# pdegenhardt/MinCostFlow

Hardware: AMD Instinct MI355X
Metric: pivots/sec + solve ms, NETGEN 100k-node/300k-arc; arc-scan GB/s vs HBM peak (higher is better)
Workload: dtype int64

## Files before the change

### include/mcf_hip.h

```cpp
#ifndef MCF_HIP_H
#define MCF_HIP_H

#include <stdint.h>

#ifdef __cplusplus
extern "C" {
#endif

#define MCF_API __attribute__((visibility("default")))

typedef enum mcf_status {
    MCF_OK = 0,
    MCF_ERR_INVALID = -1,
    MCF_ERR_NO_DEVICE = -2,
    MCF_ERR_HIP = -3,
    MCF_ERR_OVERFLOW = -4,
    MCF_ERR_TIMEOUT = -5,
    MCF_ERR_STATE = -6,
    MCF_ERR_IO = -7,
    MCF_ERR_COMM = -8
} mcf_status;

typedef enum mcf_pivot_rule { MCF_RULE_FIRST_ELIGIBLE = 0, MCF_RULE_BEST_ELIGIBLE = 1, MCF_RULE_BLOCK_SEARCH = 2,
                              MCF_RULE_CANDIDATE_LIST = 3, MCF_RULE_ALTERING_LIST = 4 } mcf_pivot_rule;
// ... 85 lines not shown
                                  const int32_t *target, const int64_t *cost);

MCF_API int mcf_engine_check_reduced_costs(mcf_engine *e, int64_t *mismatches, int32_t *first_arc);
MCF_API int mcf_engine_can_renumber(mcf_engine *e, int32_t *yes);
MCF_API int mcf_engine_renumber_nodes(mcf_engine *e, const int32_t *new_of);

MCF_API int mcf_engine_find_entering(mcf_engine *e, int32_t *found, int32_t *arc, int64_t *reduced_cost);
MCF_API int mcf_engine_search_begin(mcf_engine *e);
MCF_API int mcf_engine_search_end(mcf_engine *e, int32_t *found, int32_t *arc, int64_t *reduced_cost);

#define MCF_COLLECT_FIRST_N 0
#define MCF_COLLECT_BLOCKS 1
typedef struct mcf_collect_request {
    int32_t next_arc;
    int32_t mode;
    int32_t limit;
    int32_t block_size;
    int32_t head_length;
    int32_t survivors;
} mcf_collect_request;
MCF_API int mcf_engine_collect_eligible(mcf_engine *e, const mcf_collect_request *rq, int32_t capacity, int32_t *count, int32_t *arcs,
                                        int64_t *reduced_costs, int32_t *end_arc, int64_t *arcs_scanned);

typedef struct mcf_candidate {
    int64_t reduced_cost;
    uint32_t pos;
    int32_t arc;
    int64_t range_cost;
    uint32_t range_pos;
    int32_t range_arc;
} mcf_candidate;
MCF_API int mcf_engine_find_entering_local(mcf_engine *e, mcf_candidate *out);
MCF_API int mcf_engine_search_end_local(mcf_engine *e, mcf_candidate *out);
MCF_API int mcf_engine_resolve(mcf_engine *e, int32_t count, const mcf_candidate *all, int32_t *found,
                               int32_t *arc, int64_t *reduced_cost);
MCF_API int mcf_resolve_candidates(int32_t rule, int32_t semantics, int32_t vector_width, int32_t search_arc_num, int32_t block_size, int32_t *next_arc,
                                   int32_t count, const mcf_candidate *all, int32_t *found, int32_t *arc, int64_t *reduced_cost);
MCF_API int mcf_shard_range(int32_t search_arc_num, int32_t rank, int32_t world, int32_t *begin, int32_t *end);

MCF_API int mcf_engine_park(mcf_engine *e);
MCF_API int mcf_engine_get_next_arc(mcf_engine *e, int32_t *next_arc);
MCF_API int mcf_engine_set_next_arc(mcf_engine *e, int32_t next_arc);
MCF_API int mcf_engine_get_block_size(mcf_engine *e, int32_t *block_size);
MCF_API int mcf_engine_set_block_config(mcf_engine *e, const mcf_block_config *c, int32_t graph_node_count);

MCF_API int mcf_engine_download_pi(mcf_engine *e, int64_t *pi_out );
MCF_API int mcf_engine_download_state(mcf_engine *e, int8_t *state_out );

typedef struct mcf_engine_stats {
    int64_t searches;
    int64_t scan_launches;
    int64_t update_launches;
    int64_t inline_updates;
    int64_t potential_nodes;
    int64_t arcs_scanned;
    int64_t timed_scans;
    double timed_scan_ns;
    double host_wait_ns;
    double host_launch_ns;
    int32_t scan_workgroups, scan_threads;
    int64_t bytes_per_scan;
    int64_t resident;
    int64_t resident_launches;
    int64_t resident_requests;
    double resident_scan_ns;
    double resident_kernel_ns;
    int64_t candidates;
    int64_t host_decided;
    int64_t arcs_checked;
    int32_t initial_block_size, current_block_size;
    int32_t comm_ranks;
    int32_t reserved;
    int64_t async_refreshes;
    int64_t scan_bytes_read;
    int64_t rc_layout;
    int64_t rc_recomputes;
    int64_t renumberings;
    int64_t heap_compactions;
    int64_t rc_reloads_in_grid;
    int64_t shift_grid;
    int64_t shift_lists;
    int64_t mirror_uploads;
    double phase_shift_ns, phase_values_ns, phase_scan_ns;
} mcf_engine_stats;
MCF_API int mcf_engine_get_stats(mcf_engine *e, mcf_engine_stats *out);
MCF_API int mcf_engine_reset_stats(mcf_engine *e);

MCF_API int mcf_engine_bench_scan(mcf_engine *e, int32_t reps, int32_t cold, int64_t flush_bytes,
                                  double *avg_ns, double *min_ns);

MCF_API int mcf_engine_bench_update(mcf_engine *e, int32_t count, int32_t reps, double *avg_ns, double *min_ns, int64_t *bytes);

MCF_API int mcf_engine_bench_search(mcf_engine *e, int32_t reps, double *avg_ns, double *min_ns);

MCF_API int mcf_comm_unique_id(uint8_t id_out[128]);
MCF_API int mcf_engine_comm_init(mcf_engine *e, const uint8_t id[128], int32_t rank, int32_t world);
MCF_API int mcf_engine_find_entering_sharded(mcf_engine *e, int32_t *found, int32_t *arc, int64_t *reduced_cost);

typedef struct mcf_exchange mcf_exchange;
MCF_API int mcf_exchange_open(mcf_exchange **out, const char *name, int32_t rank, int32_t world);
MCF_API void mcf_exchange_close(mcf_exchange *x);
MCF_API int mcf_exchange_all_gather(mcf_exchange *x, const mcf_candidate *mine, mcf_candidate *all );


typedef struct mcf_ns mcf_ns;

MCF_API int mcf_ns_create(mcf_ns **out, int32_t node_count, int32_t arc_count, const int32_t *source, const int32_t *target);
MCF_API void mcf_ns_destroy(mcf_ns *s);
MCF_API int mcf_ns_set_arc_bounds(mcf_ns *s, int32_t arc, int64_t lower, int64_t upper);
MCF_API int mcf_ns_set_arc_cost(mcf_ns *s, int32_t arc, int64_t cost);
MCF_API int mcf_ns_set_node_supply(mcf_ns *s, int32_t node, int64_t supply);
MCF_API int mcf_ns_set_problem(mcf_ns *s, const int64_t *lower, const int64_t *upper, const int64_t *cost, const int64_t *supply);
MCF_API int mcf_ns_set_supply_type(mcf_ns *s, int32_t type);
MCF_API int mcf_ns_set_pivot_rule(mcf_ns *s, int32_t rule);
MCF_API int mcf_ns_set_list_pivot_rule(mcf_ns *s, int32_t rule);
MCF_API int mcf_ns_enable_optimized_pivot(mcf_ns *s, int32_t enable);
MCF_API int mcf_ns_set_vector_width(mcf_ns *s, int32_t vector_width);
MCF_API int mcf_ns_set_optimization_config(mcf_ns *s, const mcf_block_config *config);
MCF_API int mcf_ns_enable_optimizations(mcf_ns *s, int32_t flags);
MCF_API int mcf_ns_set_auto_configuration(mcf_ns *s, int32_t enable);
MCF_API int mcf_ns_set_device(mcf_ns *s, int32_t device, int32_t int_width ,
                              int32_t block_size , int32_t engine_flags);
MCF_API int mcf_ns_set_device_share(mcf_ns *s, int32_t resident_workgroups);
MCF_API int mcf_ns_set_sharding(mcf_ns *s, const uint8_t nccl_id[128], int32_t rank, int32_t world);

MCF_API int mcf_ns_set_sharding_host(mcf_ns *s, const char *exchange_name, int32_t rank, int32_t world);
MCF_API int mcf_ns_set_shard_group(mcf_ns *s, int32_t shards, const int32_t *devices);

MCF_API int mcf_ns_prepare(mcf_ns *s);
MCF_API int mcf_ns_solve(mcf_ns *s, int32_t *status);
MCF_API int mcf_ns_status(mcf_ns *s, int32_t *status);
MCF_API int mcf_ns_get_flow(mcf_ns *s, int32_t arc, int64_t *flow);
MCF_API int mcf_ns_get_potential(mcf_ns *s, int32_t node, int64_t *potential);
MCF_API int mcf_ns_get_total_cost(mcf_ns *s, int64_t *cost);
MCF_API int mcf_ns_get_flows(mcf_ns *s, int64_t *flow_out );
MCF_API int mcf_ns_get_potentials(mcf_ns *s, int64_t *pi_out );
MCF_API int mcf_ns_get_arc_upper_bound(mcf_ns *s, int32_t arc, int64_t *upper);

typedef struct mcf_ns_metrics {
    int64_t iterations;
    double total_solve_us, pivot_search_us, tree_update_us, potential_update_us;
    double setup_us;
    double loop_us;
    int32_t search_arc_num, block_size, int_width, reserved;
    int64_t degenerate_pivots;
    int64_t potential_nodes;
    mcf_engine_stats engine;
    int32_t initial_block_size, final_block_size;
    int64_t total_arcs_checked;
    double average_arcs_checked_per_pivot;
    int32_t baseline_iterations;
    int32_t config_flags;
    double iteration_ratio;
    int32_t reference_selects_cached_pivot;
    int32_t reserved2;
} mcf_ns_metrics;
MCF_API int mcf_ns_get_metrics(mcf_ns *s, mcf_ns_metrics *out);
typedef struct mcf_list_rule_stats {
    int32_t rule;
    int32_t list_length;
    int32_t minor_limit;
    int32_t block_size;
    int32_t head_length;
    int32_t reserved;
    int64_t searches;
    int64_t major_scans;
    int64_t host_answered;
    int64_t device_arcs_read;
    int64_t lemon_arcs_scanned;
// ... 430 lines not shown
```

### mincostflow_amd/_lib.py

```python
from __future__ import annotations

import ctypes as C
import importlib.util
import os
import re
import sys
import warnings

import numpy as np

_HERE = os.path.dirname(os.path.abspath(__file__))
LIB_PATH = os.path.join(_HERE, "libmcf_hip.so")

RULE_FIRST_ELIGIBLE, RULE_BEST_ELIGIBLE, RULE_BLOCK_SEARCH, RULE_CANDIDATE_LIST, RULE_ALTERING_LIST = 0, 1, 2, 3, 4
COLLECT_FIRST_N, COLLECT_BLOCKS = 0, 1
SEM_PLAIN, SEM_OPTIMIZED = 1, 2
VECTOR_DEFAULT, VECTOR_NONE = 0, -1
SUPPLY_GEQ, SUPPLY_LEQ = 0, 1
NOT_SOLVED, OPTIMAL, INFEASIBLE, UNBOUNDED, UNBALANCED = 0, 1, 2, 3, 4
STATE_UPPER, STATE_TREE, STATE_LOWER = -1, 0, 1
INF_CAP = np.iinfo(np.int64).max
ENGINE_SAMPLE_KERNEL_TIME, ENGINE_TIME_EVERY_KERNEL, ENGINE_NO_INLINE_UPDATE, ENGINE_RESIDENT, ENGINE_DISPATCH, ENGINE_CANDIDATES = 1, 2, 4, 8, 16, 32
ENGINE_SHARE_DEVICE = 64
ENGINE_NO_CANDIDATES = 128
ERR_INVALID, ERR_NO_DEVICE, ERR_HIP, ERR_OVERFLOW, ERR_TIMEOUT, ERR_STATE, ERR_IO, ERR_COMM = -1, -2, -3, -4, -5, -6, -7, -8


class McfError(RuntimeError):
    def __init__(self, code: int, message: str):
        super().__init__(f"mcf_hip error {code}: {message}")
        self.code = code


class EngineDesc(C.Structure):
    _fields_ = [(n, C.c_int32) for n in ("node_count", "arc_capacity", "search_arc_num", "int_width", "rule", "semantics",
                                         "block_size", "device", "shard_begin", "shard_end", "scan_workgroups", "flags", "resident_workgroups", "vector_width")]


class Candidate(C.Structure):
    _fields_ = [("reduced_cost", C.c_int64), ("pos", C.c_uint32), ("arc", C.c_int32),
                ("range_cost", C.c_int64), ("range_pos", C.c_uint32), ("range_arc", C.c_int32)]

    def __init__(self, reduced_cost=0, pos=0xFFFFFFFF, arc=-1, range_cost=0, range_pos=0xFFFFFFFF, range_arc=-1):
        super().__init__(reduced_cost, pos, arc, range_cost, range_pos, range_arc)


class EngineStats(C.Structure):
    _fields_ = [("searches", C.c_int64), ("scan_launches", C.c_int64), ("update_launches", C.c_int64),
                ("inline_updates", C.c_int64), ("potential_nodes", C.c_int64), ("arcs_scanned", C.c_int64),
                ("timed_scans", C.c_int64), ("timed_scan_ns", C.c_double), ("host_wait_ns", C.c_double),
                ("host_launch_ns", C.c_double), ("scan_workgroups", C.c_int32), ("scan_threads", C.c_int32),
                ("bytes_per_scan", C.c_int64), ("resident", C.c_int64), ("resident_launches", C.c_int64),
                ("resident_requests", C.c_int64), ("resident_scan_ns", C.c_double), ("resident_kernel_ns", C.c_double), ("candidates", C.c_int64),
                ("host_decided", C.c_int64), ("arcs_checked", C.c_int64), ("initial_block_size", C.c_int32), ("current_block_size", C.c_int32),
                ("comm_ranks", C.c_int32), ("reserved", C.c_int32), ("async_refreshes", C.c_int64), ("scan_bytes_read", C.c_int64), ("rc_layout", C.c_int64), ("rc_recomputes", C.c_int64), ("renumberings", C.c_int64), ("heap_compactions", C.c_int64), ("rc_reloads_in_grid", C.c_int64), ("shift_grid", C.c_int64), ("shift_lists", C.c_int64), ("mirror_uploads", C.c_int64),
                ("phase_shift_ns", C.c_double), ("phase_values_ns", C.c_double), ("phase_scan_ns", C.c_double)]

    def as_dict(self):
        return {n: getattr(self, n) for n, _ in self._fields_ if n != "reserved"}


OPT_NONE, OPT_ADAPTIVE_BLOCK_SIZE, OPT_SMALL_BLOCKS_FOR_DENSE, OPT_REDUCED_COST_CACHING = 0, 1, 2, 4


class BlockConfig(C.Structure):
    _fields_ = [("flags", C.c_int32), ("min_block_size", C.c_int32), ("max_block_size", C.c_int32), ("consecutive_hits_before_adapt", C.c_int32),
                ("min_block_size_ratio", C.c_double), ("block_size_growth_factor", C.c_double), ("block_size_shrink_factor", C.c_double),
                ("low_hit_rate_threshold", C.c_double), ("high_hit_rate_threshold", C.c_double)]

    def as_dict(self):
        return {n: getattr(self, n) for n, _ in self._fields_}


class NsMetrics(C.Structure):
    _fields_ = [("iterations", C.c_int64), ("total_solve_us", C.c_double), ("pivot_search_us", C.c_double),
                ("tree_update_us", C.c_double), ("potential_update_us", C.c_double), ("setup_us", C.c_double),
                ("loop_us", C.c_double), ("search_arc_num", C.c_int32),
                ("block_size", C.c_int32), ("int_width", C.c_int32), ("reserved", C.c_int32),
                ("degenerate_pivots", C.c_int64), ("potential_nodes", C.c_int64), ("engine", EngineStats),
                ("initial_block_size", C.c_int32), ("final_block_size", C.c_int32), ("total_arcs_checked", C.c_int64),
                ("average_arcs_checked_per_pivot", C.c_double), ("baseline_iterations", C.c_int32), ("config_flags", C.c_int32),
                ("iteration_ratio", C.c_double), ("reference_selects_cached_pivot", C.c_int32), ("reserved2", C.c_int32)]

    def as_dict(self):
        d = {n: getattr(self, n) for n, _ in self._fields_ if n not in ("engine", "reserved", "reserved2")}
        d["engine"] = self.engine.as_dict()
        return d


VALIDATION_KINDS = ("conservation", "lower", "upper", "slack_pos", "slack_neg", "node_dual", "node_slack", "objective", "dual_cost", "status")


class CollectRequest(C.Structure):
    _fields_ = [(n, C.c_int32) for n in ("next_arc", "mode", "limit", "block_size", "head_length", "survivors")]


class ListRuleStats(C.Structure):
    _fields_ = [("rule", C.c_int32), ("list_length", C.c_int32), ("minor_limit", C.c_int32), ("block_size", C.c_int32), ("head_length", C.c_int32),
                ("reserved", C.c_int32), ("searches", C.c_int64), ("major_scans", C.c_int64), ("host_answered", C.c_int64),
                ("device_arcs_read", C.c_int64), ("lemon_arcs_scanned", C.c_int64), ("collected", C.c_int64), ("collect_us", C.c_double)]

    def as_dict(self):
        return {n: getattr(self, n) for n, _ in self._fields_ if n != "reserved"}


class Validation(C.Structure):
    _fields_ = [("valid", C.c_int32), ("supply_type", C.c_int32), ("objective", C.c_int64), ("dual_cost", C.c_int64),
                ("errors", C.c_int64 * len(VALIDATION_KINDS)), ("first", C.c_int64 * len(VALIDATION_KINDS)),
                ("kernel_us", C.c_double), ("algorithmic_bytes", C.c_int64)]

    def as_dict(self):
        return {"valid": int(self.valid), "supply_type": int(self.supply_type), "objective": int(self.objective), "dual_cost": int(self.dual_cost),
                "errors": dict(zip(VALIDATION_KINDS, map(int, self.errors))), "first": dict(zip(VALIDATION_KINDS, map(int, self.first))),
                "kernel_us": float(self.kernel_us), "algorithmic_bytes": int(self.algorithmic_bytes)}


class BatchDesc(C.Structure):
    _fields_ = [("device", C.c_int32), ("pivot_rule", C.c_int32), ("semantics", C.c_int32), ("reserved", C.c_int32), ("pivot_limit", C.c_int64),
                ("pivots_per_launch", C.c_int32), ("trace_capacity", C.c_int32), ("flags", C.c_int32)]


class BatchStats(C.Structure):
    _fields_ = [("instances", C.c_int64), ("lds_instances", C.c_int64), ("global_instances", C.c_int64), ("launches", C.c_int64),
                ("total_pivots", C.c_int64), ("workspace_bytes", C.c_int64), ("lds_bytes_max", C.c_int64), ("kernel_ns", C.c_double), ("host_ns", C.c_double)]

    def as_dict(self):
        return {n: getattr(self, n) for n, _ in self._fields_}


class BatchResolveStats(C.Structure):
    _fields_ = [("warm_instances", C.c_int64), ("cold_instances", C.c_int64), ("untouched_instances", C.c_int64), ("launches", C.c_int64),
                ("total_pivots", C.c_int64), ("bytes_uploaded", C.c_int64), ("bytes_downloaded", C.c_int64), ("kernel_ns", C.c_double), ("host_ns", C.c_double)]

    def as_dict(self):
        return {n: getattr(self, n) for n, _ in self._fields_}


BATCH_MAX_ARCS, BATCH_MAX_NODES, BATCH_MAX_INSTANCES, BATCH_SHARDED = 65536, 32768, 65536, 1
MEM_HOST, MEM_DEVICE = 0, 1
# ... 119 lines not shown


class RBatchDiagnoseIo(C.Structure):
    _fields_ = UBatchDiagnoseIo._fields_


class UBatchDiagnoseStats(C.Structure):
    _fields_ = [(name, C.c_int64) for name in ("instances", "none", "feasible", "cut", "open", "bounds", "lds_instances", "global_instances", "levels",
                                               "frontier_nodes", "inc_entries")] + \
               [("kernel_ns", C.c_double), ("bytes_up", C.c_int64), ("bytes_down", C.c_int64)]

    def as_dict(self):
        return {n: getattr(self, n) for n, _ in self._fields_}


class ProblemStruct(C.Structure):
    _fields_ = [("node_count", C.c_int32), ("arc_count", C.c_int32), ("source", C.POINTER(C.c_int32)),
                ("target", C.POINTER(C.c_int32)), ("lower", C.POINTER(C.c_int64)), ("upper", C.POINTER(C.c_int64)),
                ("cost", C.POINTER(C.c_int64)), ("supply", C.POINTER(C.c_int64))]


_i32p = np.ctypeslib.ndpointer(np.int32, flags="C_CONTIGUOUS")
_i64p = np.ctypeslib.ndpointer(np.int64, flags="C_CONTIGUOUS")


class _i64p_or_null(_i64p):
    @classmethod
    def from_param(cls, obj):
        return None if obj is None else _i64p.from_param(obj)


_i8p = np.ctypeslib.ndpointer(np.int8, flags="C_CONTIGUOUS")
_u8p = np.ctypeslib.ndpointer(np.uint8, flags="C_CONTIGUOUS")
_P = C.POINTER

SIGNATURES = {
    "mcf_last_error": (C.c_char_p, []),
    "mcf_version": (C.c_char_p, []),
    "mcf_device_count": (C.c_int, []),
    "mcf_device_compute_units": (C.c_int, [C.c_int32]),
    "mcf_engine_create": (C.c_int, [_P(C.c_void_p), _P(EngineDesc)]),
    "mcf_engine_destroy": (None, [C.c_void_p]),
    "mcf_engine_upload": (C.c_int, [C.c_void_p, _i32p, _i32p, _i64p, _i8p, _i64p]),
    "mcf_engine_patch_state": (C.c_int, [C.c_void_p, C.c_int32, _i32p, _i8p]),
    "mcf_engine_update_potential": (C.c_int, [C.c_void_p, C.c_int32, _i32p, C.c_int64]),
    "mcf_engine_set_potential": (C.c_int, [C.c_void_p, C.c_int32, _i32p, _i64p]),
    "mcf_engine_append_potential": (C.c_int, [C.c_void_p, C.c_int32, _i32p, _i64p]),
    "mcf_engine_bind_potentials": (C.c_int, [C.c_void_p, C.c_void_p]),
    "mcf_engine_shift_potential": (C.c_int, [C.c_void_p, C.c_int32, _i32p, _i64p_or_null, C.c_int64]),
    "mcf_engine_shift_potential_runs": (C.c_int, [C.c_void_p, C.c_int32, _i32p, _i32p, C.c_int64]),
    "mcf_engine_reload_threshold": (C.c_int, [C.c_void_p, C.POINTER(C.c_int32)]),
    "mcf_engine_reload_potentials": (C.c_int, [C.c_void_p, C.c_int32]),
    "mcf_engine_patch_arcs": (C.c_int, [C.c_void_p, C.c_int32, _i32p, _i32p, _i32p, _i64p]),
    "mcf_engine_can_renumber": (C.c_int, [C.c_void_p, _P(C.c_int32)]),
    "mcf_engine_check_reduced_costs": (C.c_int, [C.c_void_p, _P(C.c_int64), _P(C.c_int32)]),
    "mcf_ns_check_reduced_costs": (C.c_int, [C.c_void_p, _P(C.c_int64)]),
    "mcf_engine_renumber_nodes": (C.c_int, [C.c_void_p, _i32p]),
    "mcf_engine_find_entering": (C.c_int, [C.c_void_p, _P(C.c_int32), _P(C.c_int32), _P(C.c_int64)]),
    "mcf_engine_search_begin": (C.c_int, [C.c_void_p]),
    "mcf_engine_search_end": (C.c_int, [C.c_void_p, _P(C.c_int32), _P(C.c_int32), _P(C.c_int64)]),
    "mcf_engine_find_entering_local": (C.c_int, [C.c_void_p, _P(Candidate)]),
    "mcf_engine_collect_eligible": (C.c_int, [C.c_void_p, _P(CollectRequest), C.c_int32, _P(C.c_int32), C.c_void_p, C.c_void_p,
                                              _P(C.c_int32), _P(C.c_int64)]),
    "mcf_engine_search_end_local": (C.c_int, [C.c_void_p, _P(Candidate)]),
    "mcf_exchange_open": (C.c_int, [_P(C.c_void_p), C.c_char_p, C.c_int32, C.c_int32]),
    "mcf_exchange_close": (None, [C.c_void_p]),
    "mcf_exchange_all_gather": (C.c_int, [C.c_void_p, _P(Candidate), _P(Candidate)]),
    "mcf_engine_resolve": (C.c_int, [C.c_void_p, C.c_int32, _P(Candidate), _P(C.c_int32), _P(C.c_int32), _P(C.c_int64)]),
    "mcf_resolve_candidates": (C.c_int, [C.c_int32, C.c_int32, C.c_int32, C.c_int32, C.c_int32, _P(C.c_int32), C.c_int32, _P(Candidate),
                                        _P(C.c_int32), _P(C.c_int32), _P(C.c_int64)]),
    "mcf_shard_range": (C.c_int, [C.c_int32, C.c_int32, C.c_int32, _P(C.c_int32), _P(C.c_int32)]),
    "mcf_engine_park": (C.c_int, [C.c_void_p]),
    "mcf_engine_get_next_arc": (C.c_int, [C.c_void_p, _P(C.c_int32)]),
    "mcf_engine_set_next_arc": (C.c_int, [C.c_void_p, C.c_int32]),
    "mcf_engine_get_block_size": (C.c_int, [C.c_void_p, _P(C.c_int32)]),
    "mcf_block_config_default": (None, [_P(BlockConfig)]),
    "mcf_block_config_auto": (C.c_int, [_P(BlockConfig), C.c_int32, C.c_int32, _i32p, _i32p]),
    "mcf_block_initial_size": (C.c_int, [_P(BlockConfig), C.c_int32, C.c_int32, _P(C.c_int32), _P(C.c_int32)]),
    "mcf_block_adapt": (C.c_int, [_P(BlockConfig), C.c_int32, C.c_int64, _P(C.c_int32), _P(C.c_int32)]),
    "mcf_engine_set_block_config": (C.c_int, [C.c_void_p, _P(BlockConfig), C.c_int32]),
    "mcf_engine_download_pi": (C.c_int, [C.c_void_p, _i64p]),
    "mcf_engine_download_state": (C.c_int, [C.c_void_p, _i8p]),
    "mcf_engine_get_stats": (C.c_int, [C.c_void_p, _P(EngineStats)]),
    "mcf_engine_reset_stats": (C.c_int, [C.c_void_p]),
    "mcf_engine_bench_scan": (C.c_int, [C.c_void_p, C.c_int32, C.c_int32, C.c_int64, _P(C.c_double), _P(C.c_double)]),
    "mcf_engine_bench_search": (C.c_int, [C.c_void_p, C.c_int32, _P(C.c_double), _P(C.c_double)]),
    "mcf_engine_bench_update": (C.c_int, [C.c_void_p, C.c_int32, C.c_int32, _P(C.c_double), _P(C.c_double), _P(C.c_int64)]),
    "mcf_comm_unique_id": (C.c_int, [_u8p]),
    "mcf_engine_comm_init": (C.c_int, [C.c_void_p, _u8p, C.c_int32, C.c_int32]),
    "mcf_engine_find_entering_sharded": (C.c_int, [C.c_void_p, _P(C.c_int32), _P(C.c_int32), _P(C.c_int64)]),
    "mcf_ns_create": (C.c_int, [_P(C.c_void_p), C.c_int32, C.c_int32, _i32p, _i32p]),
    "mcf_ns_destroy": (None, [C.c_void_p]),
    "mcf_ns_set_arc_bounds": (C.c_int, [C.c_void_p, C.c_int32, C.c_int64, C.c_int64]),
    "mcf_ns_set_arc_cost": (C.c_int, [C.c_void_p, C.c_int32, C.c_int64]),
    "mcf_ns_set_node_supply": (C.c_int, [C.c_void_p, C.c_int32, C.c_int64]),
    "mcf_ns_set_problem": (C.c_int, [C.c_void_p, C.c_void_p, C.c_void_p, C.c_void_p, C.c_void_p]),
    "mcf_ns_set_supply_type": (C.c_int, [C.c_void_p, C.c_int32]),
    "mcf_ns_set_pivot_rule": (C.c_int, [C.c_void_p, C.c_int32]),
    "mcf_ns_set_list_pivot_rule": (C.c_int, [C.c_void_p, C.c_int32]),
    "mcf_ns_enable_optimized_pivot": (C.c_int, [C.c_void_p, C.c_int32]),
    "mcf_ns_set_vector_width": (C.c_int, [C.c_void_p, C.c_int32]),
    "mcf_ns_set_optimization_config": (C.c_int, [C.c_void_p, _P(BlockConfig)]),
    "mcf_ns_enable_optimizations": (C.c_int, [C.c_void_p, C.c_int32]),
    "mcf_ns_set_auto_configuration": (C.c_int, [C.c_void_p, C.c_int32]),
    "mcf_ns_set_device": (C.c_int, [C.c_void_p, C.c_int32, C.c_int32, C.c_int32, C.c_int32]),
    "mcf_ns_set_device_share": (C.c_int, [C.c_void_p, C.c_int32]),
    "mcf_ns_set_sharding": (C.c_int, [C.c_void_p, _u8p, C.c_int32, C.c_int32]),
    "mcf_ns_set_sharding_host": (C.c_int, [C.c_void_p, C.c_char_p, C.c_int32, C.c_int32]),
    "mcf_ns_set_shard_group": (C.c_int, [C.c_void_p, C.c_int32, _i32p]),
    "mcf_ns_prepare": (C.c_int, [C.c_void_p]),
    "mcf_ns_solve": (C.c_int, [C.c_void_p, _P(C.c_int32)]),
    "mcf_ns_status": (C.c_int, [C.c_void_p, _P(C.c_int32)]),
    "mcf_ns_get_flow": (C.c_int, [C.c_void_p, C.c_int32, _P(C.c_int64)]),
    "mcf_ns_get_potential": (C.c_int, [C.c_void_p, C.c_int32, _P(C.c_int64)]),
    "mcf_ns_get_total_cost": (C.c_int, [C.c_void_p, _P(C.c_int64)]),
    "mcf_ns_get_flows": (C.c_int, [C.c_void_p, _i64p]),
    "mcf_ns_get_potentials": (C.c_int, [C.c_void_p, _i64p]),
    "mcf_ns_get_arc_upper_bound": (C.c_int, [C.c_void_p, C.c_int32, _P(C.c_int64)]),
    "mcf_ns_get_metrics": (C.c_int, [C.c_void_p, _P(NsMetrics)]),
    "mcf_ns_get_list_rule_stats": (C.c_int, [C.c_void_p, _P(ListRuleStats)]),
    "mcf_ns_set_pivot_limit": (C.c_int, [C.c_void_p, C.c_int64]),
    "mcf_ns_set_trace": (C.c_int, [C.c_void_p, C.c_void_p, C.c_int64]),
    "mcf_ns_get_trace_length": (C.c_int, [C.c_void_p, _P(C.c_int64)]),
    "mcf_ns_begin": (C.c_int, [C.c_void_p, _P(C.c_int32)]),
    "mcf_ns_apply_pivot": (C.c_int, [C.c_void_p, C.c_int32, _P(C.c_int32)]),
    "mcf_ns_finish": (C.c_int, [C.c_void_p, _P(C.c_int32)]),
    "mcf_ns_replay": (C.c_int, [C.c_void_p, _i32p, C.c_int64, C.c_int32, C.c_double]),
    "mcf_ns_check_thread_breaks": (C.c_int, [C.c_void_p, _P(C.c_int64)]),
    "mcf_ns_internal": (C.c_int, [C.c_void_p, _P(C.c_int32), _P(C.c_int32), _P(_P(C.c_int32)), _P(_P(C.c_int32)),
                                  _P(_P(C.c_int64)), _P(_P(C.c_int8)), _P(_P(C.c_int64))]),
    "mcf_ns_tree": (C.c_int, [C.c_void_p, _P(_P(C.c_int32)), _P(_P(C.c_int32)), _P(_P(C.c_int32)), _P(_P(C.c_int8)), _P(_P(C.c_int64)), _P(_P(C.c_int64))]),
    "mcf_ns_last_pivot": (C.c_int, [C.c_void_p, _P(C.c_int32), _P(C.c_int32), _P(C.c_int8), _P(C.c_int32),
                                    _P(_P(C.c_int32)), _P(C.c_int64)]),
    "mcf_validator_create": (C.c_int, [_P(C.c_void_p), C.c_int32, C.c_int32, C.c_int32]),
    "mcf_validator_destroy": (None, [C.c_void_p]),
    "mcf_validator_upload": (C.c_int, [C.c_void_p] + [C.c_void_p] * 8),
    "mcf_validator_run": (C.c_int, [C.c_void_p, C.c_int32, C.c_int64, _P(Validation)]),
    "mcf_ns_validate": (C.c_int, [C.c_void_p, _P(Validation)]),
    "mcf_batch_create": (C.c_int, [_P(C.c_void_p), _P(BatchDesc)]),
    "mcf_batch_destroy": (None, [C.c_void_p]),
    "mcf_batch_add": (C.c_int, [C.c_void_p, C.c_int32, C.c_int32, C.c_void_p, C.c_void_p, C.c_void_p, C.c_void_p, C.c_void_p, C.c_void_p, C.c_int32, _P(C.c_int32)]),
    "mcf_batch_solve": (C.c_int, [C.c_void_p]),
    "mcf_batch_run_on_host": (C.c_int, [C.c_void_p]),
    "mcf_batch_get_status": (C.c_int, [C.c_void_p, C.c_int32, _P(C.c_int32)]),
    "mcf_batch_get_total_cost": (C.c_int, [C.c_void_p, C.c_int32, _P(C.c_int64)]),
    "mcf_batch_get_flows": (C.c_int, [C.c_void_p, C.c_int32, C.c_void_p]),
    "mcf_batch_get_potentials": (C.c_int, [C.c_void_p, C.c_int32, C.c_void_p]),
    "mcf_batch_get_pivots": (C.c_int, [C.c_void_p, C.c_int32, _P(C.c_int64)]),
    "mcf_batch_get_trace": (C.c_int, [C.c_void_p, C.c_int32, C.c_void_p, C.c_int64, _P(C.c_int64)]),
    "mcf_batch_get_stats": (C.c_int, [C.c_void_p, _P(BatchStats)]),
    "mcf_batch_set_costs": (C.c_int, [C.c_void_p, C.c_int32, C.c_void_p]),
    "mcf_batch_resolve": (C.c_int, [C.c_void_p]),
    "mcf_batch_rerun_on_host": (C.c_int, [C.c_void_p]),
    "mcf_batch_get_resolve_stats": (C.c_int, [C.c_void_p, _P(BatchResolveStats)]),
    "mcf_ubatch_create": (C.c_int, [_P(C.c_void_p), _P(UBatchDesc)]),
    "mcf_ubatch_destroy": (None, [C.c_void_p]),
    "mcf_ubatch_solve": (C.c_int, [C.c_void_p, _P(UBatchIo)]),
    "mcf_ubatch_resolve": (C.c_int, [C.c_void_p, _P(UBatchIo)]),
    "mcf_ubatch_run_on_host": (C.c_int, [C.c_void_p, _P(UBatchIo)]),
    "mcf_ubatch_rerun_on_host": (C.c_int, [C.c_void_p, _P(UBatchIo)]),
    "mcf_ubatch_get_stats": (C.c_int, [C.c_void_p, _P(UBatchStats)]),
    "mcf_ubatch_resolve_data": (C.c_int, [C.c_void_p, _P(UBatchIo)]),
    "mcf_ubatch_rerun_data_on_host": (C.c_int, [C.c_void_p, _P(UBatchIo)]),
    "mcf_ubatch_get_redata_stats": (C.c_int, [C.c_void_p, _P(UBatchRedataStats)]),
    "mcf_ubatch_validate": (C.c_int, [C.c_void_p, _P(UBatchCheckIo), _P(UBatchCheckSummary)]),
    "mcf_ubatch_validate_on_host": (C.c_int, [C.c_void_p, _P(UBatchCheckIo), _P(UBatchCheckSummary)]),
# ... 105 lines not shown
```

### mincostflow_amd/csrc/candidate_cache.hip.h

```cpp
#pragma once

static_assert(kCandNone == kNone, "the state's 'no arc' is the kernels'");
constexpr int kCandRefreshLow = 12;
constexpr int kCandMaxAvgDegree = 24;

inline const int64_t *cand_pi(const mcf_engine *e) { return e->ext_pi ? e->ext_pi : e->pi.data(); }
inline CandGraph cand_graph(const mcf_engine *e)
{
    return CandGraph{e->adj_start.data(), e->adj.data(), e->h_src.data(), e->h_tgt.data(), e->h_cost.data(), e->h_state.data(), cand_pi(e)};
}

inline void cand_note_node(mcf_engine *e, int u, bool sigma_known = false, int64_t sigma = 0)
{
    if (e->rc_mode) {
        if (sigma_known) e->rc_sync.push_back(mcf_engine::NodeShift{u, sigma});
        else e->rc_shift_unknown = true;
    }
    if (e->blind_count > 0 && e->blind_epoch == e->cand_now) e->blind_sets = 2;
    if (cand_state_note_node(e, u, e->adj_start.data())) e->sync_nodes.push_back(u);
}
inline void cand_note_arc(mcf_engine *e, int a)
{
    if (cand_state_note_arc(e, a)) e->sync_arcs.push_back(a);
}
// ... 26 lines not shown
        for (int r = 0; r < n_runs; ++r) for (int k = 0; k < length[r]; ++k) e->pend_node.push_back(first[r] + k);
        e->pend_val.resize(e->pend_node.size(), 0);
        e->blind_count = e->pend_node.size();
    } else {
        e->blind_lazy = true;
        for (int r = 0; r < n_runs; ++r)
            for (int32_t at = 0; at < length[r]; at += kShiftRunMax) {
                e->blind_runs.push_back((uint32_t)(first[r] + at));
                e->blind_runs.push_back((uint32_t)std::min<int32_t>(kShiftRunMax, length[r] - at));
            }
        e->blind_count += (size_t)total;
    }
    if (e->async_posted && cand_records_ready(e, 0)) { const int rc = cand_collect(e, e->async_at); if (rc) return rc; }
    shift_stream(e);
    return MCF_OK;
}

inline int cand_note_nodes_blind(mcf_engine *e, int32_t count, const int32_t *nodes, const int64_t *values, bool continuation)
{
    if (e->blind_lazy) {
        if (e->shift_streamed > 0) { const int rc = resident_stop(e); if (rc) return rc; }
        cand_materialise_blind(e);
    }
    e->pivot_overflow = true;
    if (e->blind_count == 0) { e->blind_epoch = e->cand_now; e->blind_sets = 0; }
    if (!continuation) {
        e->blind_sets += 1;
        if (e->blind_sets > 1 && e->stream_lines > 0) { const int rc = resident_stop(e); if (rc) return rc; }
    }
    e->pend_node.insert(e->pend_node.end(), nodes, nodes + count);
    if (values) e->pend_val.insert(e->pend_val.end(), values, values + count);
    else {
        const size_t at = e->pend_val.size();
        e->pend_val.resize(at + (size_t)count);
        if (!e->shift_grid) for (int i = 0; i < count; ++i) e->pend_val[at + i] = e->ext_pi[nodes[i]];
    }
    e->blind_count = e->pend_node.size();
    if (e->async_posted && cand_records_ready(e, 0)) { const int rc = cand_collect(e, e->async_at); if (rc) return rc; }
    if (e->shift_grid) shift_stream(e);
    else resident_stream(e);
    return MCF_OK;
}

bool cand_decide(mcf_engine *e, Key *k)
{
    mcf_engine::CandKey win;
    if (!cand_decide(static_cast<CandState *>(e), &win)) return false;
    k->c = win.p == kNone ? 0 : win.c;
    k->r = 0;
    k->p = win.p;
    return true;
}

int cand_build_patches(mcf_engine *e)
{
    const int64_t *pi = cand_pi(e);
    const size_t n_b = e->blind_count, n_s = e->sync_nodes.size();
    const bool blind_current = n_b == 0 || (e->blind_epoch == e->cand_now && e->blind_sets <= 1);
    const bool squeeze = (int64_t)n_b + (int64_t)n_s > e->patch_capacity;
    if ((!blind_current || squeeze) && e->stream_lines > 0) { const int rc = resident_stop(e); if (rc) return rc; }
    if (squeeze) {
        e->pend_node.insert(e->pend_node.end(), e->sync_nodes.begin(), e->sync_nodes.end());
        std::sort(e->pend_node.begin(), e->pend_node.end());
        e->pend_node.erase(std::unique(e->pend_node.begin(), e->pend_node.end()), e->pend_node.end());
        e->pend_val.resize(e->pend_node.size());
        for (size_t i = 0; i < e->pend_node.size(); ++i) e->pend_val[i] = pi[e->pend_node[i]];
    } else {
        if (!blind_current) for (size_t i = 0; i < n_b; ++i) e->pend_val[i] = pi[e->pend_node[i]];
        e->pend_node.resize(n_b + n_s);
        e->pend_val.resize(n_b + n_s);
        for (size_t i = 0; i < n_s; ++i) { e->pend_node[n_b + i] = e->sync_nodes[i]; e->pend_val[n_b + i] = pi[e->sync_nodes[i]]; }
    }
    e->pend_arc.assign(e->sync_arcs.begin(), e->sync_arcs.end());
    e->pend_state.resize(e->pend_arc.size());
    for (size_t i = 0; i < e->pend_arc.size(); ++i) e->pend_state[i] = e->h_state[e->pend_arc[i]];
    e->sync_nodes.clear();
    e->sync_arcs.clear();
    blind_clear(e);
    e->rc_sync.clear();
    e->rc_shift_unknown = false;
    return MCF_OK;
}

bool cand_records_ready(const mcf_engine *e, int g)
{
    const volatile Slot *rec = e->h_slots + (size_t)g * kCandRecords;
    for (int r = 0; r < kCandRecords; ++r) { const int64_t c = rec[r].c; const uint32_t q = rec[r].p; if (rec[r].tag != record_tag(e->seq, c, q)) return false; }
    return true;
}

int cand_collect(mcf_engine *e, uint32_t at)
{
    const double t0 = (double)__rdtsc();
    double t0_wall = 0;
    const volatile Slot *slots = e->h_slots;
    e->cand_records.clear();
    mcf_engine::CandKey thr{0, kNone};
    for (int g = 0; g < e->res_grid; ++g) {
        const volatile Slot *rec = slots + (size_t)g * kCandRecords;
        uint64_t spins = 0;
        while (!cand_records_ready(e, g)) {
            _mm_pause();
            if (e->resident_running && (spins & 0xFFF) == 0xFFF && ((const volatile uint32_t *)e->h_exit)[0] != 0) {
                if (((const volatile uint32_t *)e->h_exit)[0] == kExitPartial) {
                    (void)resident_join(e, false);
                    e->resident_running = false;
                    resident_slot_release(e);
                    return mcf::fail(MCF_ERR_TIMEOUT, "the resident grid could not meet at its grid-wide barrier while a list was being applied (are its workgroups all resident?): the device arrays are undefined");
                }
                int rc = resident_restart(e);
                if (rc) return rc;
            }
            if ((++spins & 0xFFFFF) == 0) {
                const hipError_t q = hipStreamQuery(e->res_stream ? e->res_stream : e->stream);
                if (q != hipSuccess && q != hipErrorNotReady) return mcf::fail(MCF_ERR_HIP, "resident grid failed: %s", hipGetErrorString(q));
                if (t0_wall == 0) t0_wall = mcf::now_ns();
                else if (mcf::now_ns() - t0_wall > 20e9) return mcf::fail(MCF_ERR_TIMEOUT, "no answer from the device after 20 s (workgroup %d of %d)", g, e->res_grid);
            }
        }
        std::atomic_thread_fence(std::memory_order_acquire);
        for (int r = 0; r < kCandPerGroup; ++r)
            if (rec[r].p != kNone) e->cand_records.push_back(mcf_engine::CandKey{rec[r].c, rec[r].p});
        if (rec[kCandPerGroup].p != kNone) {
            const mcf_engine::CandKey t{rec[kCandPerGroup].c, rec[kCandPerGroup].p};
            if (thr.p == kNone || cand_key_less(t, thr)) thr = t;
        }
    }
    e->wait_ticks += (double)__rdtsc() - t0;
    cand_install(e, cand_graph(e), e->cand_records.data(), e->cand_records.size(), thr, at);
    e->tk_collect += (double)__rdtsc() - t0;
    return MCF_OK;
}

int cand_post_rc(mcf_engine *e)
{
    const bool reload = e->reload_pi && e->d_ext_pi != nullptr && (int64_t)e->sync_arcs.size() <= e->mailbox_max_st;
    if (reload) {
        pend_clear_potentials(e);
        e->sync_nodes.clear(); e->rc_sync.clear(); e->rc_shift_unknown = false;
        blind_clear(e);
        e->reload_pi = false;
    }
    const size_t n_b = e->blind_count, n_s = e->rc_sync.size();
    const bool blind_ok = n_b == 0 || (e->pend_shift && e->blind_epoch == e->cand_now);
    const int64_t n_st = (int64_t)e->sync_arcs.size();
    const bool fast = !e->reload_pi && !e->rc_shift_unknown && blind_ok && (int64_t)(n_b + n_s) <= (int64_t)e->rc_list_max && n_st <= e->mailbox_max_st;
    if (fast) {
        e->pend_node.resize(n_b + n_s);
        e->pend_val.resize(n_b + n_s);
        for (size_t i = 0; i < n_b; ++i) e->pend_val[i] = e->pend_sigma;
        for (size_t i = 0; i < n_s; ++i) { e->pend_node[n_b + i] = e->rc_sync[i].node; e->pend_val[n_b + i] = e->rc_sync[i].shift; }
        e->pend_arc.assign(e->sync_arcs.begin(), e->sync_arcs.end());
        e->pend_state.resize(e->pend_arc.size());
        for (size_t i = 0; i < e->pend_arc.size(); ++i) e->pend_state[i] = e->h_state[e->pend_arc[i]];
        e->sync_nodes.clear(); e->sync_arcs.clear(); e->rc_sync.clear();
        blind_clear(e);
    } else {
        if (int rcb = cand_build_patches(e)) return rcb;
        int rc = resident_stop(e);
        if (!rc) rc = flush_pending(e);
        if (rc) return rc;
    }
    next_request_keep_prev(e);
    int rc = resident_start(e, e->prev_seq);
    if (rc) return rc;
    resident_post(e, e->seq, reload ? kCmdReload : kCmdScan, fast);
    if (reload) e->st.rc_reloads_in_grid += 1;
    if (fast && (!e->pend_node.empty() || !e->pend_arc.empty())) e->st.inline_updates += 1;
    pend_clear(e);
    e->posted_at = e->cand_now;
    e->st.arcs_scanned += e->end - e->begin;
    return MCF_OK;
}


int device_sync_from_mirrors(mcf_engine *e)
{
    const int64_t *pi = cand_pi(e);
    HIP_TRY(hipMemcpyAsync(e->d_pi, pi, sizeof(int64_t) * (size_t)e->d.node_count, hipMemcpyHostToDevice, e->stream));
    HIP_TRY(hipMemcpyAsync(e->d_state, e->h_state.data() + e->begin, (size_t)(e->end - e->begin), hipMemcpyHostToDevice, e->stream));
    HIP_TRY(hipStreamSynchronize(e->stream));
    pend_clear(e);
    e->pend_shift = false;
    e->sync_nodes.clear(); e->sync_arcs.clear(); e->rc_sync.clear(); e->rc_shift_unknown = false;
    blind_clear(e); e->blind_sets = 0;
    e->shift_streamed = 0;
    e->reload_pi = false;
    e->st.mirror_uploads += 1;
    return MCF_OK;
}

void shift_write_lines(mcf_engine *e, int from, int to, size_t n, bool runs, uint32_t seq)
{
    const int per_line = runs ? kShiftPairsPerLine : kShiftNodesPerLine;
    MailboxLine line;
    for (int l = from; l < to; ++l) {
        memset(line.w, 0, sizeof(line.w));
        for (int k = 0; k < per_line && (size_t)l * per_line + k < n; ++k) {
            const size_t i = (size_t)l * per_line + k;
            if (runs) { line.w[2 * k] = e->blind_runs[2 * i]; line.w[2 * k + 1] = e->blind_runs[2 * i + 1]; }
            else line.w[k] = (uint32_t)e->pend_node[i];
        }
        line.w[15] = seq;
        mailbox_write_line(e->mailbox + e->shift_base + 16 * (size_t)l, line.w);
    }
}

void shift_post_request(mcf_engine *e, uint32_t seq, uint32_t cmd, size_t val_lo, size_t n_shift, int64_t sigma, bool with_patches, bool runs = false)
{
    const int n_val = with_patches ? (int)(e->pend_node.size() - val_lo) : 0, n_st = with_patches ? (int)e->pend_arc.size() : 0;
    const ValueEntries vals{e->pend_node.data(), e->pend_val.data(), val_lo + 1, n_val > 1 ? n_val - 1 : 0};
    const StateEntries sts{e->pend_arc.data(), e->pend_state.data(), 2, n_st > 2 ? n_st - 2 : 0};
    const MailboxLine line1 = mailbox_encode_entries(e->mailbox, vals, sts, seq);
    if (with_patches) {
        const int per_line = runs ? kShiftPairsPerLine : kShiftNodesPerLine;
        shift_write_lines(e, e->shift_streamed, (int)((n_shift + per_line - 1) / per_line), n_shift, runs, seq);
        e->shift_streamed = 0;
    }
    MailboxLine h = request_header(e, seq, cmd, n_st, n_val, val_lo);
    h.w[kShHdrValues] = (uint32_t)n_val;
    h.w[kShHdrShift] = with_patches ? (uint32_t)n_shift : 0u;
    h.w[kShHdrRuns] = with_patches && runs ? 1u : 0u;
    h.w[kShHdrSigma] = (uint32_t)(uint64_t)sigma;
    h.w[kShHdrSigma + 1] = (uint32_t)((uint64_t)sigma >> 32);
    mailbox_publish(e->mailbox, kPollReplicas, h, vals.n + sts.n > 0 ? &line1 : nullptr);
}
void shift_post(mcf_engine *e, uint32_t seq, uint32_t cmd, bool) { shift_post_request(e, seq, cmd, 0, 0, 0, false); }

constexpr int kShiftStreamMinLines = 96;
void shift_stream(mcf_engine *e)
{
    if (e->async_posted || e->blind_epoch != e->cand_now || e->blind_sets > 1 || !e->pend_shift) return;
    if (!e->resident_running || e->in_flight != mcf_engine::kNoSearch) return;
    const bool runs = e->blind_lazy;
    const int complete = runs ? (int)(e->blind_runs.size() / 2 / kShiftPairsPerLine) : (int)(e->blind_count / kShiftNodesPerLine);
    if (complete - e->shift_streamed < kShiftStreamMinLines || complete > e->max_shift_lines) return;
    const uint32_t next_seq = peek_request(e);
    shift_write_lines(e, e->shift_streamed, complete, runs ? e->blind_runs.size() / 2 : e->blind_count, runs, next_seq);
    e->stream_sub += 1;
    if (e->stream_sub == 0) e->stream_sub = 1;
    MailboxLine h = request_header(e, next_seq, runs ? kCmdApplyRuns : kCmdApply);
    h.w[kShHdrShift] = (uint32_t)complete;
    h.w[kShHdrApplySub] = e->stream_sub;
    mailbox_publish(e->mailbox, kPollReplicas, h, nullptr);
    e->shift_streamed = complete;
    e->stream_lines = complete;
}

int cand_post_shift(mcf_engine *e)
{
    if (!e->resident_running) {
        const int rc = resident_start(e, e->seq);
        if (rc) return rc;
    }
    if (e->reload_pi) {
        if (!e->d_ext_pi || e->shift_streamed > 0 || (int64_t)e->sync_arcs.size() > (int64_t)e->mailbox_max_st) {
            int rc = resident_stop(e);
            if (!rc) rc = resident_start(e, e->seq);
            if (rc) return rc;
        }
    }
    if (e->reload_pi) {
        pend_clear_potentials(e);
        e->sync_nodes.clear();
        blind_clear(e);
        e->pend_arc.assign(e->sync_arcs.begin(), e->sync_arcs.end());
        e->pend_state.resize(e->pend_arc.size());
        for (size_t i = 0; i < e->pend_arc.size(); ++i) e->pend_state[i] = e->h_state[e->pend_arc[i]];
        next_request_keep_prev(e);
        shift_post_request(e, e->seq, kCmdReload, 0, 0, 0, true);
        e->st.rc_reloads_in_grid += 1;
        e->pend_arc.clear(); e->pend_state.clear();
        e->sync_arcs.clear();
        e->stream_lines = 0;
        e->reload_pi = false;
        e->posted_at = e->cand_now;
        e->st.arcs_scanned += e->end - e->begin;
        return MCF_OK;
    }
    for (int attempt = 0; attempt < 2; ++attempt) {
        const size_t n_b = e->blind_count, n_s = e->sync_nodes.size();
        const bool blind_current = n_b == 0 || (e->blind_epoch == e->cand_now && e->blind_sets <= 1);
        const size_t n_pairs = e->blind_lazy ? e->blind_runs.size() / 2 : 0;
        const bool as_shift = n_b > 0 && blind_current && e->pend_shift &&
                              (e->blind_lazy ? n_pairs <= (size_t)e->max_shift_lines * kShiftPairsPerLine : n_b <= (size_t)e->max_shift_lines * kShiftNodesPerLine);
        const bool fits = (int64_t)(as_shift ? n_s : n_b + n_s) <= (int64_t)e->patch_capacity && (int64_t)e->sync_arcs.size() <= (int64_t)e->mailbox_max_st;
        if ((!as_shift && e->shift_streamed > 0) || !fits) {
            int rc = resident_stop(e);
            if (!rc) rc = resident_start(e, e->seq);
            if (rc) return rc;
            continue;
        }
        const int64_t *pi = cand_pi(e);
        const bool runs = as_shift && e->blind_lazy;
        if (!as_shift) cand_materialise_blind(e);
        const size_t base = runs ? 0 : n_b, val_lo = as_shift ? base : 0;
        if (!as_shift) for (size_t i = 0; i < n_b; ++i) e->pend_val[i] = pi[e->pend_node[i]];
        e->pend_node.resize(base + n_s);
        e->pend_val.resize(base + n_s);
        for (size_t i = 0; i < n_s; ++i) { e->pend_node[base + i] = e->sync_nodes[i]; e->pend_val[base + i] = pi[e->sync_nodes[i]]; }
        e->pend_arc.assign(e->sync_arcs.begin(), e->sync_arcs.end());
        e->pend_state.resize(e->pend_arc.size());
        for (size_t i = 0; i < e->pend_arc.size(); ++i) e->pend_state[i] = e->h_state[e->pend_arc[i]];
        next_request_keep_prev(e);
        shift_post_request(e, e->seq, kCmdScan, val_lo, as_shift ? (runs ? n_pairs : n_b) : 0, e->pend_sigma, true, runs);
        if (!e->pend_node.empty() || !e->pend_arc.empty()) e->st.inline_updates += 1;
        if (as_shift) e->st.shift_lists += 1;
        pend_clear(e);
        e->sync_nodes.clear(); e->sync_arcs.clear();
        blind_clear(e);
        e->stream_lines = 0;
        e->posted_at = e->cand_now;
        e->st.arcs_scanned += e->end - e->begin;
        return MCF_OK;
    }
    return mcf::fail(MCF_ERR_STATE, "cand_post_shift: the request does not fit an empty mailbox");
}

int cand_post(mcf_engine *e)
{
    if (e->shift_grid) return cand_post_shift(e);
    if (e->rc_mode) return cand_post_rc(e);
    if (int rcb = cand_build_patches(e)) return rcb;
    if ((int)e->pend_arc.size() > e->mailbox_max_st) {
        int rc = resident_stop(e);
        if (!rc) rc = flush_pending(e);
        if (rc) return rc;
    }
    next_request_keep_prev(e);
    int rc = resident_start(e, e->prev_seq);
    if (rc) return rc;
    resident_post(e, e->seq, kCmdScan, true);
    if (!e->pend_node.empty() || !e->pend_arc.empty()) e->st.inline_updates += 1;
    pend_clear(e);
    e->posted_at = e->cand_now;
    e->st.arcs_scanned += e->end - e->begin;
    return MCF_OK;
}

void cand_build_adjacency(mcf_engine *e)
{
    const int n = e->d.node_count, m_s = e->d.search_arc_num;
    const int32_t *source = e->h_src.data(), *target = e->h_tgt.data();
    const int lo = e->begin, hi = std::min(e->end, m_s);
    e->adj_start.assign(n + 1, 0);
    for (int a = lo; a < hi; ++a) { e->adj_start[source[a] + 1]++; if (target[a] != source[a]) e->adj_start[target[a] + 1]++; }
    for (int u = 0; u < n; ++u) e->adj_start[u + 1] += e->adj_start[u];
    e->adj.assign(e->adj_start[n], mcf_engine::AdjEnt{0, 0u, 0});
    e->adj_pos.assign((size_t)2 * m_s, -1);
    std::vector<int32_t> fill(e->adj_start.begin(), e->adj_start.end() - 1);
    for (int a = lo; a < hi; ++a) {
        const uint32_t st_bits = (uint32_t)(e->h_state[a] + 1) << 29;
        e->adj_pos[2 * (size_t)a] = fill[source[a]];
        e->adj[fill[source[a]]++] = mcf_engine::AdjEnt{a, (uint32_t)target[a] | st_bits, e->h_cost[a]};
        if (target[a] != source[a]) {
            e->adj_pos[2 * (size_t)a + 1] = fill[target[a]];
            e->adj[fill[target[a]]++] = mcf_engine::AdjEnt{a, (uint32_t)source[a] | st_bits | 0x80000000u, e->h_cost[a]};
        }
    }
}
```

### mincostflow_amd/csrc/candidate_state.h

```cpp
#pragma once

#include <algorithm>
#include <cstdint>
#include <vector>

#include "common.h"

constexpr uint32_t kCandNone = 0xFFFFFFFFu;
constexpr int kCandMaxNodes = 256;
constexpr int64_t kCandDegreePerNode = 8;

struct CandState {
    struct AdjEnt { int32_t arc; uint32_t other; int64_t cost; };
    struct CandKey { int64_t c; uint32_t p; };
    struct HeapEnt { int64_t c; uint32_t p; uint32_t at; int32_t u, v; };

    bool cand_valid = false;
    mcf::hvec<uint32_t> node_at, arc_at;
    uint32_t cand_now = 1;
    uint32_t snap_at = 0;
    uint32_t heap_gap = 0;
    std::vector<HeapEnt> heap;
    std::vector<int32_t> pivot_nodes, pivot_arcs;
    int64_t pivot_degree = 0;
    bool pivot_overflow = false;
    std::vector<CandKey> cand_list;
    std::vector<int32_t> cand_ends;
    size_t cand_ptr = 0;
    bool tp_ok = false, hd_ok = false;
    int32_t tp_a = -1, tp_u = -1, tp_v = -1, hd_a = -1, hd_u = -1, hd_v = -1;
    uint32_t tp_at = 0;
    size_t hd_ptr = 0;
    CandKey cand_thr{0, kCandNone};
    bool async_posted = false;
    size_t heap_compact_above = 1u << 18;
    int64_t n_heap_push = 0, n_heap_admit = 0, n_heap_pop = 0, n_heap_sweeps = 0;
};

struct CandGraph {
    const int32_t *adj_start;
    const CandState::AdjEnt *adj;
    const int32_t *src, *tgt;
    const int64_t *cost;
    const int8_t *state;
    const int64_t *pi;
};

inline bool cand_key_less(const CandState::CandKey &a, const CandState::CandKey &b) { return a.c < b.c || (a.c == b.c && a.p < b.p); }
struct CandHeapAfter {
    bool operator()(const CandState::HeapEnt &a, const CandState::HeapEnt &b) const { return b.c < a.c || (b.c == a.c && b.p < a.p); }
};

inline bool cand_state_note_node(CandState *e, int u, const int32_t *adj_start)
{
    if ((u == e->tp_u) | (u == e->tp_v)) e->tp_ok = false;
    if ((u == e->hd_u) | (u == e->hd_v)) e->hd_ok = false;
    if (e->node_at[u] == e->cand_now) return false;
    e->node_at[u] = e->cand_now;
    if (!e->pivot_overflow) {
        e->pivot_nodes.push_back(u);
        e->pivot_degree += adj_start[u + 1] - adj_start[u];
        if ((int)e->pivot_nodes.size() > kCandMaxNodes || e->pivot_degree > kCandDegreePerNode * kCandMaxNodes) e->pivot_overflow = true;
    }
    return true;
}
inline bool cand_state_note_arc(CandState *e, int a)
{
    if (a == e->tp_a) e->tp_ok = false;
    if (a == e->hd_a) e->hd_ok = false;
    if (e->arc_at[a] == e->cand_now) return false;
    e->arc_at[a] = e->cand_now;
    e->pivot_arcs.push_back(a);
    return true;
}

inline bool cand_heap_current(const CandState *e, const CandState::HeapEnt &t)
{
    return ((int)(e->arc_at[t.p] <= t.at) & (int)(e->node_at[t.u] <= t.at) & (int)(e->node_at[t.v] <= t.at)) != 0;
}

inline bool cand_admit_all(const CandState *e) { return e->async_posted || !e->cand_valid || e->cand_thr.p == kCandNone; }

inline void cand_sweep_heap(CandState *e, bool install)
{
    if (e->heap.empty()) return;
    size_t keep = 0;
    if (install) {
        const bool all = e->cand_thr.p == kCandNone;
        for (size_t i = 0; i < e->heap.size(); ++i) {
            const CandState::HeapEnt &t = e->heap[i];
            if (t.at > e->snap_at && (all || cand_key_less(CandState::CandKey{t.c, t.p}, e->cand_thr))) e->heap[keep++] = t;
        }
    } else {
        for (size_t i = 0; i < e->heap.size(); ++i)
            if (cand_heap_current(e, e->heap[i])) e->heap[keep++] = e->heap[i];
    }
    e->heap.resize(keep);
    std::make_heap(e->heap.begin(), e->heap.end(), CandHeapAfter());
    e->n_heap_sweeps += 1;
}

inline void cand_push(CandState *e, const CandGraph &g, int a)
{
    const int st = g.state[a];
    if (st == 0) return;
    const int64_t *pi = g.pi;
    const int32_t u = g.src[a], v = g.tgt[a];
    const int64_t d = g.cost[a] + pi[u] - pi[v];
    const int64_t rc = st > 0 ? d : -d;
    if (rc >= 0) return;
    e->n_heap_push += 1;
    if (!cand_admit_all(e) && !cand_key_less(CandState::CandKey{rc, (uint32_t)a}, e->cand_thr)) return;
    e->n_heap_admit += 1;
    e->heap.push_back(CandState::HeapEnt{rc, (uint32_t)a, e->cand_now, u, v});
    std::push_heap(e->heap.begin(), e->heap.end(), CandHeapAfter());
}

inline void cand_absorb_pivot(CandState *e, const CandGraph &g)
{
    if (e->pivot_overflow) {
// ... 2 lines not shown
        const int64_t *pi = g.pi;
        const uint32_t now = e->cand_now;
        const bool admit_all = cand_admit_all(e);
        const CandState::CandKey thr = e->cand_thr;
        int64_t offered = 0, admitted = 0;
        for (int u : e->pivot_nodes)
            for (int i = g.adj_start[u], hi = g.adj_start[u + 1]; i < hi; ++i) {
                const CandState::AdjEnt &x = g.adj[i];
                __builtin_prefetch(&pi[x.other & 0x1FFFFFFFu]);
            }
        for (int u : e->pivot_nodes) {
            const int64_t pu = pi[u];
            for (int i = g.adj_start[u], hi = g.adj_start[u + 1]; i < hi; ++i) {
                const CandState::AdjEnt &x = g.adj[i];
                const int st = (int)((x.other >> 29) & 3u) - 1;
                if (st == 0) continue;
                const int32_t other = (int32_t)(x.other & 0x1FFFFFFFu);
                const int64_t po = pi[other];
                const int64_t d = (x.other >> 31) ? x.cost + po - pu : x.cost + pu - po;
                const int64_t rc = st > 0 ? d : -d;
                if (rc >= 0) continue;
                offered += 1;
                if (!admit_all && !cand_key_less(CandState::CandKey{rc, (uint32_t)x.arc}, thr)) continue;
                admitted += 1;
                e->heap.push_back(CandState::HeapEnt{rc, (uint32_t)x.arc, now, u, other});
                std::push_heap(e->heap.begin(), e->heap.end(), CandHeapAfter());
            }
        }
        e->n_heap_push += offered;
        e->n_heap_admit += admitted;
        for (int a : e->pivot_arcs) cand_push(e, g, a);
    }
    e->pivot_nodes.clear();
    e->pivot_arcs.clear();
    e->pivot_degree = 0;
    e->pivot_overflow = false;
    if (e->heap.size() > e->heap_compact_above) cand_sweep_heap(e, false);
}

inline bool cand_decide(CandState *e, CandState::CandKey *out)
{
    if (!e->cand_valid || e->snap_at < e->heap_gap) return false;
    CandState::CandKey best_d{0, kCandNone};
    while (!e->heap.empty()) {
        const CandState::HeapEnt &t = e->heap.front();
        const uint32_t a = t.p;
        if (e->tp_ok && (int32_t)a == e->tp_a && t.at == e->tp_at) { best_d = CandState::CandKey{t.c, a}; break; }
        const bool after = t.at > e->snap_at;
        if (after && cand_heap_current(e, t)) {
            e->tp_ok = true; e->tp_a = (int32_t)a; e->tp_at = t.at; e->tp_u = t.u; e->tp_v = t.v;
            best_d = CandState::CandKey{t.c, a};
            break;
        }
        std::pop_heap(e->heap.begin(), e->heap.end(), CandHeapAfter());
        e->heap.pop_back();
        e->n_heap_pop += 1;
    }
    while (e->cand_ptr < e->cand_list.size()) {
        if (e->hd_ok && e->hd_ptr == e->cand_ptr) break;
        const uint32_t a = e->cand_list[e->cand_ptr].p;
        if (e->cand_ptr + 1 < e->cand_list.size()) {
            __builtin_prefetch(&e->arc_at[e->cand_list[e->cand_ptr + 1].p]);
            __builtin_prefetch(&e->node_at[e->cand_ends[2 * e->cand_ptr + 2]]);
            __builtin_prefetch(&e->node_at[e->cand_ends[2 * e->cand_ptr + 3]]);
        }
        const uint32_t t_arc = e->arc_at[a], t_src = e->node_at[e->cand_ends[2 * e->cand_ptr]], t_tgt = e->node_at[e->cand_ends[2 * e->cand_ptr + 1]];
        if ((t_arc <= e->snap_at) & (t_src <= e->snap_at) & (t_tgt <= e->snap_at)) {
            e->hd_ok = true; e->hd_ptr = e->cand_ptr; e->hd_a = (int32_t)a; e->hd_u = e->cand_ends[2 * e->cand_ptr]; e->hd_v = e->cand_ends[2 * e->cand_ptr + 1];
            break;
        }
        e->cand_ptr++;
    }
    CandState::CandKey win{0, kCandNone};
    if (e->cand_ptr < e->cand_list.size()) {
        win = e->cand_list[e->cand_ptr];
        if (best_d.p != kCandNone && cand_key_less(best_d, win)) win = best_d;
    } else if (e->cand_thr.p == kCandNone) {
        win = best_d;
    } else if (best_d.p != kCandNone && cand_key_less(best_d, e->cand_thr)) {
        win = best_d;
    } else {
        return false;
    }
    *out = win;
    return true;
}

inline void cand_install(CandState *e, const CandGraph &g, const CandState::CandKey *rec, size_t n, CandState::CandKey thr, uint32_t at)
{
    e->cand_thr = thr;
    e->cand_list.clear();
    for (size_t i = 0; i < n; ++i)
        if (thr.p == kCandNone || cand_key_less(rec[i], thr)) e->cand_list.push_back(rec[i]);
    std::sort(e->cand_list.begin(), e->cand_list.end(), cand_key_less);
    e->cand_ends.resize(2 * e->cand_list.size());
    for (size_t i = 0; i < e->cand_list.size(); ++i) { e->cand_ends[2 * i] = g.src[e->cand_list[i].p]; e->cand_ends[2 * i + 1] = g.tgt[e->cand_list[i].p]; }
    e->cand_ptr = 0;
    e->cand_valid = true;
    e->hd_ok = e->tp_ok = false;
    e->snap_at = at;
    e->async_posted = false;
    cand_sweep_heap(e, true);
}

inline void cand_reset(CandState *e)
{
    e->cand_valid = false;
    e->cand_list.clear();
    e->cand_ptr = 0;
    e->hd_ok = e->tp_ok = false;
    e->heap.clear();
    e->pivot_nodes.clear(); e->pivot_arcs.clear(); e->pivot_degree = 0; e->pivot_overflow = false;
    e->heap_gap = e->cand_now;
}

constexpr uint32_t kCandEpochWrap = 0xFFFFFF00u;
inline void cand_restart_epochs(CandState *e)
{
    std::fill(e->node_at.begin(), e->node_at.end(), 0u);
    std::fill(e->arc_at.begin(), e->arc_at.end(), 0u);
    const bool overflow = e->pivot_overflow;
    const std::vector<int32_t> pn = e->pivot_nodes, pa = e->pivot_arcs;
    cand_reset(e);
    e->cand_now = 1;
    e->snap_at = 0;
    e->heap_gap = 1;
    e->pivot_overflow = overflow;
    for (int u : pn) e->node_at[u] = 1;
    for (int a : pa) e->arc_at[a] = 1;
}

inline void cand_renumber(CandState *e, const int32_t *new_of, int n)
{
    mcf::hvec<uint32_t> at((size_t)n);
    for (int u = 0; u < n; ++u) at[new_of[u]] = e->node_at[u];
    std::copy(at.begin(), at.end(), e->node_at.begin());
    for (size_t i = 0; i < e->cand_ends.size(); ++i) e->cand_ends[i] = new_of[e->cand_ends[i]];
    for (auto &h : e->heap) { h.u = new_of[h.u]; h.v = new_of[h.v]; }
    e->tp_ok = e->hd_ok = false;
    for (int32_t &u : e->pivot_nodes) u = new_of[u];
}
```

### mincostflow_amd/csrc/engine.hip

```cpp
#include <hip/hip_runtime.h>
#include <hip/hip_ext.h>
#include <hsa/hsa.h>
#include <hsa/hsa_ext_amd.h>

#include <dlfcn.h>
#include <immintrin.h>

#include <algorithm>
#include <atomic>
#include <cmath>
#include <cstdio>
#include <cstring>
#include <map>
#include <mutex>
#include <vector>

#include "common.h"
#include "candidate_state.h"

#include "kernels.hip.h"
#include "collect.hip.h"

namespace {

// ... 76 lines not shown
    int rc_recompute_above = INT32_MAX;
    int rc_list_max = 0;
    bool pend_shift = false;
    int64_t pend_sigma = 0;
    bool no_pireg = false;
    int lds_grid = 0;
    uint32_t seq = 0;
    bool uploaded = false;
    mcf::hvec<int64_t> pi;
    bool mirror_valid = false;
    bool ext_pi_pinned = false;
    const int64_t *d_ext_pi = nullptr;
    uint32_t *d_barrier = nullptr;
    int32_t *d_node_map = nullptr;
    bool reload_pi = false;
    const int64_t *ext_pi = nullptr;
    int64_t max_abs_cost = 0;
    mcf::hvec<int32_t> pend_node, pend_arc, pend_state;
    mcf::hvec<int64_t> pend_val;
    struct Staging {
        int32_t *nodes = nullptr, *arcs = nullptr, *states = nullptr;
        int64_t *values = nullptr;
        void *d_nodes = nullptr, *d_arcs = nullptr, *d_states = nullptr, *d_values = nullptr;
        hipEvent_t done = nullptr;
        bool busy = false;
        int cap_nodes = 0;
    } stage[2];
    int stage_next = 0;
    static constexpr int kEvRing = 64;
    hipEvent_t ev_start[kEvRing]{}, ev_stop[kEvRing]{};
    int ev_head = 0, ev_tail = 0;
    mcf_engine_stats st{};
    void *comm = nullptr;
    int rank = 0, world = 1;
    mcf_candidate *d_cand_local = nullptr, *d_cand_all = nullptr, *h_cand_all = nullptr;
    struct XRec { uint64_t head; mcf_candidate c; uint64_t pad[2]; uint64_t tail; };
    XRec *x_send = nullptr, *x_recv = nullptr;
    void *d_x_send = nullptr, *d_x_recv = nullptr;
    hipStream_t comm_stream = nullptr;
    uint64_t x_seq = 0;
    bool comm_resident = false;
    bool resident_ok = false, resident_running = false, resident_reg = false;
    bool has_slot = false;
    int shift_reload_min = 0;
    bool shift_grid = false;
    uint32_t shift_base = 0;
    int max_shift_lines = 0;
    int cand_tiles = 1;
    int shift_streamed = 0;
    double wait_ticks = 0, launch_ticks = 0, cal_ns = 0, cal_ticks = 0;
    enum { kNoSearch = 0, kAnswered, kResidentSearch, kCandSearch, kDispatchSearch } in_flight = kNoSearch;
    Key answered{0, kNone, kNone};
    Key range_key{0, kNone, kNone};
    int vec = 0;
    bool in_flight_timed = false;
    int stream_lines = 0;
    uint32_t stream_sub = 0;
    uint32_t *mailbox = nullptr;
    int mailbox_lines = 0, mailbox_max_st = 0;
    uint32_t idle_ticks = 0;
    uint32_t prev_seq = 0;
    bool cand_on = false;
    mcf::hvec<int32_t> h_src, h_tgt;
    mcf::hvec<int64_t> h_cost;
    mcf::hvec<int8_t> h_state;
    mcf::hvec<int32_t> adj_start;
    mcf::hvec<AdjEnt> adj;
    mcf::hvec<int32_t> adj_pos;
    std::vector<int32_t> sync_nodes, sync_arcs;
    size_t blind_count = 0;
    std::vector<uint32_t> blind_runs;
    bool blind_lazy = false;
    uint32_t blind_epoch = 0;
    int blind_sets = 0;
    bool force_device_search = false;
    bool cand_appending = false;
    struct NodeShift { int32_t node; int64_t shift; };
    std::vector<NodeShift> rc_sync;
    bool rc_shift_unknown = false;
    bool call_shift_known = false;
    int64_t call_shift = 0;
    std::vector<CandState::CandKey> cand_records;
    uint32_t async_at = 0, posted_at = 0;
    int patch_capacity = 0;
    uint32_t cand_epoch0 = 1;
    bool cand_debug = false;
    double tk_absorb = 0, tk_decide = 0, tk_post = 0, tk_collect = 0, tk_probe = 0;
    int64_t n_sync_posts = 0, n_async_waits = 0, n_gap_pivots = 0, n_list_skip = 0;
    uint32_t *h_exit = nullptr, *d_exit = nullptr;
    int res_grid = 0, res_threads = kResidentThreads;
    hipEvent_t res_start = nullptr, res_stop = nullptr;
    void *d_flush = nullptr;
    size_t flush_bytes = 0;
    bool list_rule = false;
    std::vector<int32_t> pend_index;
    CollectTile *d_tiles = nullptr;
    CollectHeader *h_collect_hdr = nullptr, *d_collect_hdr = nullptr;
    CollectEntry *h_collect = nullptr, *d_collect = nullptr;
    int collect_cap = 0;
};

namespace {
inline void blind_clear(mcf_engine *e)
{
    e->blind_count = 0;
    e->blind_runs.clear();
    e->blind_lazy = false;
}

#include "engine_helpers.hip.h"

bool fits32(int64_t v) { return v >= INT32_MIN && v <= INT32_MAX; }

int drain_events(mcf_engine *e, bool all)
{
    while (e->ev_tail != e->ev_head) {
        const int i = e->ev_tail % mcf_engine::kEvRing;
        if (!all && hipEventQuery(e->ev_stop[i]) != hipSuccess) break;
        HIP_TRY(hipEventSynchronize(e->ev_stop[i]));
        float ms = 0.f;
        HIP_TRY(hipEventElapsedTime(&ms, e->ev_start[i], e->ev_stop[i]));
        e->st.timed_scans += 1;
        e->st.timed_scan_ns += (double)ms * 1e6;
        e->ev_tail++;
    }
    return MCF_OK;
}

template <typename T>
void fill_params(mcf_engine *e, ScanParams<T> &p, bool with_patches)
{
    p.src = e->d_src;
    p.tgt = e->d_tgt;
    p.cost = (const T *)e->d_cost;
    p.state = e->d_state;
    p.pi = (T *)e->d_pi;
    p.slots = e->slots_target ? e->slots_target : e->d_slots;
    p.orig = e->bucket_nodes > 0 ? e->d_orig : nullptr;
    p.base = e->begin;
    p.count_padded = e->count_padded;
    p.m_s = e->d.search_arc_num;
    const SearchHeader h = search_header(e);
    p.next_arc = h.next_arc;
    p.block_size = h.block_size;
    p.rstar = h.rstar;
    p.seq = e->seq;
    p.n_pi = 0;
    p.n_st = 0;
    if (with_patches) {
        p.n_pi = (int)e->pend_node.size();
        p.n_st = (int)e->pend_arc.size();
        for (int i = 0; i < p.n_pi; ++i) { p.pi_node[i] = e->pend_node[i]; p.pi_val[i] = (T)e->pend_val[i]; }
        for (int i = 0; i < p.n_st; ++i) { p.st_arc[i] = e->pend_arc[i]; p.st_val[i] = e->pend_state[i]; }
    }
}

void fill_rc_params(mcf_engine *e, RcParams &p, bool with_states)
{
    p.state_ro = e->d_state; p.state = e->d_state; p.rc = e->d_rc; p.slots = e->slots_target ? e->slots_target : e->d_slots;
    p.base = e->begin; p.count_padded = e->count_padded; p.m_s = e->d.search_arc_num;
    const SearchHeader h = search_header(e);
    p.next_arc = h.next_arc;
    p.block_size = h.block_size;
    p.rstar = h.rstar;
    p.seq = e->seq;
    p.n_st = 0;
// ... 408 lines not shown
    if (desc->int_width != 32 && desc->int_width != 64) return mcf::fail(MCF_ERR_INVALID, "int_width must be 32 or 64");
    if (desc->rule < 0 || desc->rule > 4) return mcf::fail(MCF_ERR_INVALID, "pivot rule %d does not exist (Types/PivotRule.cs:7-41)", desc->rule);
    const bool list_rule = desc->rule == MCF_RULE_CANDIDATE_LIST || desc->rule == MCF_RULE_ALTERING_LIST;
    if (list_rule && !((desc->shard_begin == 0 && desc->shard_end == 0) || (desc->shard_begin == 0 && desc->shard_end == desc->search_arc_num)))
        return mcf::fail(MCF_ERR_INVALID, "the list rules (3, 4) scan the whole search range: no arc shards");
    if (desc->semantics != MCF_SEM_PLAIN && desc->semantics != MCF_SEM_OPTIMIZED) return mcf::fail(MCF_ERR_INVALID, "bad semantics %d", desc->semantics);
    if (desc->vector_width != MCF_VECTOR_DEFAULT && desc->vector_width != MCF_VECTOR_NONE && desc->vector_width != 2 && desc->vector_width != 4 && desc->vector_width != 8)
        return mcf::fail(MCF_ERR_INVALID, "vector_width %d is not Vector<long>.Count of any machine (2, 4, 8, MCF_VECTOR_NONE, or 0 = 4)", desc->vector_width);
    if (mcf_device_count() <= desc->device || desc->device < 0)
        return mcf::fail(MCF_ERR_NO_DEVICE, "HIP device %d not available (%d visible); this library has no CPU search path", desc->device, mcf_device_count());
    HIP_TRY(hipSetDevice(desc->device));
    mcf_engine *e = new mcf_engine();
    e->cal_ns = mcf::now_ns();
    e->cal_ticks = (double)__rdtsc();
    e->d = *desc;
    e->list_rule = list_rule;
    e->vec = desc->vector_width == MCF_VECTOR_NONE ? 0 : (desc->vector_width == MCF_VECTOR_DEFAULT ? 4 : desc->vector_width);
    e->begin = desc->shard_begin;
    e->end = desc->shard_end;
    if (e->begin == 0 && e->end == 0) e->end = desc->search_arc_num;
    if (e->begin < 0 || e->end < e->begin || e->end > desc->search_arc_num || (e->begin % kArcsPerThread) != 0) {
        delete e;
        return mcf::fail(MCF_ERR_INVALID, "bad shard [%d, %d)", desc->shard_begin, desc->shard_end);
    }
    const int count = e->end - e->begin;
    {
        const int64_t groups4 = ((int64_t)count + kArcsPerThread - 1) / kArcsPerThread;
        const int max_grid = desc->resident_workgroups > 0 ? std::min(desc->resident_workgroups, kResidentMaxGrid) : kResidentMaxGrid;
        int g = (int)std::min<int64_t>(max_grid, std::max<int64_t>(1, (groups4 + 255) / 256));
        int64_t t = ((groups4 + g - 1) / g + 63) / 64 * 64;
        t = std::max<int64_t>(64, std::min<int64_t>(t, kResidentThreads));
        e->res_grid = g;
        e->res_threads = (int)t;
        e->resident_reg = (int64_t)g * t * kArcsPerThread >= count;
    }
    e->count_padded = std::max(kPad, (count + kPad - 1) / kPad * kPad);
    if (e->resident_reg) {
        const int64_t need = (int64_t)e->res_grid * e->res_threads * kArcsPerThread;
        if (need > e->count_padded) e->count_padded = (int)((need + kPad - 1) / kPad * kPad);
    }
    e->block_size = desc->block_size > 0 ? desc->block_size : mcf::default_block_size(desc->search_arc_num, desc->semantics);
    e->unroll = count > (1 << 20) ? 2 : 1;
    const int groups = e->count_padded / (kTile * e->unroll);
    e->grid = desc->scan_workgroups > 0 ? std::min(desc->scan_workgroups, kMaxWorkgroups) : std::min(groups, kScanMaxGrid);
    e->grid = std::max(1, std::min(e->grid, groups));
    e->lds_pi = desc->node_count <= kLdsPiMax;
    e->no_pireg = (desc->flags & MCF_ENGINE_SHARE_DEVICE) != 0;
    if (e->lds_pi) {
        e->unroll = count > (2 << 20) ? 2 : 1;
        const int tiles = e->count_padded / (e->unroll * kResidentTile);
        e->grid = std::max(1, std::min(tiles, desc->scan_workgroups > 0 ? desc->scan_workgroups : 256));
    }
    {
        bool want = !e->resident_reg && !e->lds_pi;
        want = mcf::env_int("MCF_HIP_RC", 0, 1, want) != 0;
        if (list_rule) want = false;
        e->rc_mode = want;
        if (e->rc_mode) {
            e->rc_recompute_above = std::max(1024, desc->node_count / 16);
            e->rc_list_max = kRcResidentNodes;
            const int recompute = (int)mcf::env_int("MCF_HIP_RC_RECOMPUTE", 0, INT32_MAX, e->rc_recompute_above);
            e->rc_recompute_above = recompute == 0 ? INT32_MAX : recompute;
            e->unroll = count > (1 << 20) ? 2 : 1;
            const int groups_rc = std::max(1, e->count_padded / (kThreads * kArcsPerThread * e->unroll));
            e->grid = desc->scan_workgroups > 0 ? std::min(desc->scan_workgroups, kMaxWorkgroups) : std::min(groups_rc, kRcMaxGrid);
            e->grid = std::max(1, std::min(e->grid, groups_rc));
        }
    }
    e->patch_capacity = 2 * desc->node_count + 256;
    const size_t w = desc->int_width / 8;
    hipError_t err = hipSuccess;
    auto chk = [&](hipError_t x) { if (err == hipSuccess && x != hipSuccess) err = x; };
    chk(hipStreamCreateWithFlags(&e->stream, hipStreamNonBlocking));
    chk(hipMalloc((void **)&e->d_src, sizeof(int32_t) * e->count_padded));
    chk(hipMalloc((void **)&e->d_tgt, sizeof(int32_t) * e->count_padded));
    chk(hipMalloc(&e->d_cost, w * e->count_padded));
    chk(hipMalloc((void **)&e->d_state, e->count_padded));
    chk(hipMalloc(&e->d_pi, w * (size_t)desc->node_count));
    if (e->rc_mode) {
        chk(hipMalloc((void **)&e->d_rc, sizeof(int64_t) * e->count_padded));
        chk(hipMalloc((void **)&e->d_adj_start, sizeof(int32_t) * ((size_t)desc->node_count + 1)));
        chk(hipMalloc((void **)&e->d_adj, sizeof(uint32_t) * (size_t)std::max(1, 2 * count)));
    }
    chk(hipHostMalloc((void **)&e->h_slots, sizeof(Slot) * kMaxWorkgroups * kSlotStride, hipHostMallocMapped | hipHostMallocCoherent));
    if (err == hipSuccess) {
        memset(e->h_slots, 0, sizeof(Slot) * kMaxWorkgroups * kSlotStride);
        chk(hipHostGetDevicePointer((void **)&e->d_slots, e->h_slots, 0));
    }
    for (int i = 0; i < 2 && err == hipSuccess; ++i) {
        mcf_engine::Staging &s = e->stage[i];
        s.cap_nodes = 2 * desc->node_count + 256;
        chk(hipHostMalloc((void **)&s.nodes, sizeof(int32_t) * s.cap_nodes, hipHostMallocMapped | hipHostMallocCoherent));
        chk(hipHostMalloc((void **)&s.values, sizeof(int64_t) * s.cap_nodes, hipHostMallocMapped | hipHostMallocCoherent));
        chk(hipHostMalloc((void **)&s.arcs, sizeof(int32_t) * kStageStates, hipHostMallocMapped | hipHostMallocCoherent));
        chk(hipHostMalloc((void **)&s.states, sizeof(int32_t) * kStageStates, hipHostMallocMapped | hipHostMallocCoherent));
        if (err == hipSuccess) {
            chk(hipHostGetDevicePointer(&s.d_nodes, s.nodes, 0));
            chk(hipHostGetDevicePointer(&s.d_values, s.values, 0));
            chk(hipHostGetDevicePointer(&s.d_arcs, s.arcs, 0));
            chk(hipHostGetDevicePointer(&s.d_states, s.states, 0));
        }
        chk(hipEventCreateWithFlags(&s.done, hipEventDisableTiming));
    }
    for (int i = 0; i < mcf_engine::kEvRing && err == hipSuccess; ++i) { chk(hipEventCreate(&e->ev_start[i])); chk(hipEventCreate(&e->ev_stop[i])); }
    if (list_rule && err == hipSuccess) {
        e->pend_index.assign((size_t)desc->node_count, -1);
        chk(hipMalloc((void **)&e->d_tiles, sizeof(CollectTile) * kCollectMaxTiles));
        chk(hipHostMalloc((void **)&e->h_collect_hdr, sizeof(CollectHeader), hipHostMallocMapped | hipHostMallocCoherent));
        if (err == hipSuccess) chk(hipHostGetDevicePointer((void **)&e->d_collect_hdr, e->h_collect_hdr, 0));
    }
    if (err != hipSuccess) {
        const int rc = mcf::fail(MCF_ERR_HIP, "mcf_engine_create: %s", hipGetErrorString(err));
        mcf_engine_destroy(e);
        return rc;
    }
    {
        const int env = (int)mcf::env_int("MCF_HIP_RESIDENT", 0, 1, -1);
        bool want = (desc->flags & MCF_ENGINE_DISPATCH) == 0;
        if (!e->resident_reg && !e->lds_pi) want = false;
        if (e->rc_mode) want = (desc->flags & MCF_ENGINE_DISPATCH) == 0;
        if (env == 1 && !e->rc_mode) want = true;
        if (env == 0) want = false;
        if (list_rule) want = false;
        if (want && !(desc->flags & (MCF_ENGINE_TIME_EVERY_KERNEL | MCF_ENGINE_NO_INLINE_UPDATE))) {
            e->mailbox_max_st = 4096;
            e->mailbox_lines = 2 + (e->patch_capacity + e->mailbox_max_st + kMailboxPatchesPerLine - 1) / kMailboxPatchesPerLine;
            e->max_shift_lines = (desc->node_count + kShiftNodesPerLine - 1) / kShiftNodesPerLine + 1;
            e->shift_base = (uint32_t)kMailboxTail + 16u * (uint32_t)e->mailbox_lines;
            e->idle_ticks = (uint32_t)(mcf::env_int("MCF_HIP_IDLE_MS", 1, 10000, kResidentIdleTicks / 100000) * 100000);
            e->mailbox = alloc_bar_vram(desc->device, (size_t)kMailboxTail * 4 + ((size_t)e->mailbox_lines + e->max_shift_lines) * 64);
            if (e->mailbox && hipHostMalloc((void **)&e->h_exit, 64, hipHostMallocMapped | hipHostMallocCoherent) == hipSuccess &&
                hipHostGetDevicePointer((void **)&e->d_exit, e->h_exit, 0) == hipSuccess &&
                hipEventCreate(&e->res_start) == hipSuccess && hipEventCreate(&e->res_stop) == hipSuccess) {
                alignas(16) uint32_t zero[16] = {0};
                for (size_t l = 0; l < (size_t)kMailboxTail / 16 + e->mailbox_lines + e->max_shift_lines; ++l) mailbox_write_line(e->mailbox + 16 * l, zero);
                _mm_sfence();
                e->resident_ok = true;
                if (e->rc_mode) {
                    const int max_grid = desc->resident_workgroups > 0 ? std::min(desc->resident_workgroups, kResidentMaxGrid) : kResidentMaxGrid;
                    e->res_threads = kResidentThreads;
                    e->res_grid = std::max(1, std::min(max_grid, e->count_padded / kResidentTile));
                    const int64_t per = ((int64_t)e->count_padded + e->res_grid - 1) / e->res_grid;
                    e->rc_window = (int)((per + kResidentTile - 1) / kResidentTile * kResidentTile);
                    e->rc_lds = e->rc_window <= kRcWindow && !mcf::env_off("MCF_HIP_RC_LDS");
                    if (!e->rc_lds) e->rc_window = 0;
                    e->resident_reg = false;
                    if (hipMalloc((void **)&e->d_barrier, 64) != hipSuccess) { e->d_barrier = nullptr; (void)hipGetLastError(); }
                    e->rc_list_max = e->d_barrier ? std::min(2 * desc->node_count, std::max(kRcResidentNodes, e->rc_recompute_above)) : kRcResidentNodes;
                }
                e->cand_on = !(desc->flags & MCF_ENGINE_NO_CANDIDATES) && !mcf::env_off("MCF_HIP_CANDIDATES") &&
                             (e->resident_reg || e->rc_mode) && desc->rule == MCF_RULE_BEST_ELIGIBLE && desc->node_count < (1 << 29) &&
                             2 * (int64_t)desc->search_arc_num <= (int64_t)kCandMaxAvgDegree * desc->node_count;
                e->shift_grid = e->cand_on && e->resident_reg && !e->rc_mode && !e->lds_pi && !e->no_pireg && desc->int_width == 64 &&
                                desc->node_count <= kShiftBits;
                if (e->shift_grid) {
                    const int64_t groups4 = ((int64_t)count + kArcsPerThread - 1) / kArcsPerThread;
                    e->cand_tiles = groups4 <= (int64_t)2 * e->res_grid * kCandThreads ? 2 : 4;
                    const int64_t t = std::max<int64_t>(64, ((groups4 + (int64_t)e->cand_tiles * e->res_grid - 1) / ((int64_t)e->cand_tiles * e->res_grid) + 63) / 64 * 64);
                    if (t > kCandThreads) e->shift_grid = false;
                    else e->res_threads = (int)t;
                }
                if (e->shift_grid) {
                    e->shift_reload_min = (int)mcf::env_int("MCF_HIP_SHIFT_RELOAD", 0, INT32_MAX, 32768);
                    if (e->shift_reload_min > 0 && hipMalloc((void **)&e->d_barrier, 64) != hipSuccess) { e->d_barrier = nullptr; (void)hipGetLastError(); }
                }
            }
        }
    }
    e->st.scan_workgroups = e->resident_ok ? e->res_grid : e->grid;
    {
        int want = (count >= kBucketMinArcs && desc->node_count > 2 * kBucketNodes) ? kBucketNodes : 0;
        want = (int)mcf::env_int("MCF_HIP_BUCKET_NODES", 0, INT32_MAX, want);
        const bool tile_loop = !e->lds_pi && !(e->resident_ok && e->resident_reg) && !e->rc_mode;
        if (want > 0 && desc->rule == MCF_RULE_BEST_ELIGIBLE && tile_loop && !e->cand_on) {
            if (hipMalloc((void **)&e->d_orig, sizeof(int32_t) * e->count_padded) == hipSuccess) e->bucket_nodes = want;
        }
    }
    e->st.scan_threads = e->resident_ok ? e->res_threads : (e->lds_pi ? kResidentThreads : kThreads);
    e->st.resident = e->resident_ok ? 1 : 0;
    e->st.candidates = e->cand_on ? 1 : 0;
    e->st.bytes_per_scan = (int64_t)(desc->int_width == 64 ? 17 : 13) * count + (int64_t)w * desc->node_count;
    e->st.scan_bytes_read = e->rc_mode ? (int64_t)9 * count : e->st.bytes_per_scan;
    e->st.rc_layout = e->rc_mode ? 1 : 0;
    e->st.shift_grid = e->shift_grid ? 1 : 0;
    e->st.initial_block_size = e->st.current_block_size = e->block_size;
    e->cand_epoch0 = (uint32_t)mcf::env_int("MCF_HIP_CAND_EPOCH0", 1, 0xFFFFFFFFll, 1);
    e->heap_compact_above = (size_t)mcf::env_int("MCF_HIP_CAND_HEAP_COMPACT", 1, 1ll << 30, (long long)e->heap_compact_above);
    e->cand_debug = getenv("MCF_HIP_CAND_DEBUG") != nullptr;
    *out = e;
    return MCF_OK;
}

namespace {
std::mutex g_pin_mutex;
std::map<const void *, int> g_pins;
bool host_pin(const void *p, size_t bytes)
{
    std::lock_guard<std::mutex> lock(g_pin_mutex);
    auto it = g_pins.find(p);
    if (it != g_pins.end()) { it->second += 1; return true; }
    const hipError_t r = hipHostRegister(const_cast<void *>(p), bytes, hipHostRegisterPortable | hipHostRegisterMapped);
    (void)hipGetLastError();
    if (r != hipSuccess) return false;
    g_pins[p] = 1;
    return true;
}
void host_unpin(const void *p)
{
    std::lock_guard<std::mutex> lock(g_pin_mutex);
    auto it = g_pins.find(p);
    if (it == g_pins.end()) return;
    if (--it->second > 0) return;
    g_pins.erase(it);
    (void)hipHostUnregister(const_cast<void *>(p));
    (void)hipGetLastError();
}
}

void mcf_engine_destroy(mcf_engine *e)
{
    if (!e) return;
    if (e->cand_on && e->cand_debug && e->st.searches > 1000) {
        const double ns_per_tick = (mcf::now_ns() - e->cal_ns) / std::max(1.0, (double)__rdtsc() - e->cal_ticks);
        const double n = (double)e->st.searches;
        fprintf(stderr, "[cand] searches %lld host %lld async %lld sync_posts %lld async_waits %lld gap_pivots %lld | per search ns: absorb %.0f probe %.0f decide %.0f post %.0f collect %.0f wait %.0f | heap size %zu pushes %lld admitted %lld pops %lld sweeps %lld\n",
                (long long)e->st.searches, (long long)e->st.host_decided, (long long)e->st.async_refreshes, (long long)e->n_sync_posts, (long long)e->n_async_waits,
                (long long)e->n_gap_pivots, e->tk_absorb * ns_per_tick / n, e->tk_probe * ns_per_tick / n, e->tk_decide * ns_per_tick / n, e->tk_post * ns_per_tick / n,
                e->tk_collect * ns_per_tick / n, e->wait_ticks * ns_per_tick / n, e->heap.size(), (long long)e->n_heap_push, (long long)e->n_heap_admit, (long long)e->n_heap_pop,
                (long long)e->n_heap_sweeps);
    }
    (void)hipSetDevice(e->d.device);
    (void)resident_stop(e);
    if (e->ext_pi && e->ext_pi_pinned) { if (e->stream) (void)hipStreamSynchronize(e->stream); host_unpin(e->ext_pi); }
    if (e->stream) (void)hipStreamSynchronize(e->stream);
    if (e->res_stream) { (void)hipStreamSynchronize(e->res_stream); (void)hipStreamDestroy(e->res_stream); e->res_stream = nullptr; }
    if (e->mailbox) hsa_amd_memory_pool_free(e->mailbox);
    if (e->h_exit) (void)hipHostFree(e->h_exit);
    if (e->res_start) (void)hipEventDestroy(e->res_start);
    if (e->res_stop) (void)hipEventDestroy(e->res_stop);
    if (e->comm && rccl() && rccl()->comm_destroy) rccl()->comm_destroy(e->comm);
    if (e->d_orig) (void)hipFree(e->d_orig);
    (void)hipFree(e->d_rc); (void)hipFree(e->d_adj_start); (void)hipFree(e->d_adj); (void)hipFree(e->d_barrier); (void)hipFree(e->d_node_map);
    (void)hipFree(e->d_src); (void)hipFree(e->d_tgt); (void)hipFree(e->d_cost); (void)hipFree(e->d_state); (void)hipFree(e->d_pi);
    (void)hipFree(e->d_cand_local); (void)hipFree(e->d_cand_all); (void)hipFree(e->d_flush); (void)hipFree(e->d_dev_slots);
    (void)hipFree(e->d_tiles);
    if (e->h_collect_hdr) (void)hipHostFree(e->h_collect_hdr);
    if (e->h_collect) (void)hipHostFree(e->h_collect);
    if (e->h_cand_all) (void)hipHostFree(e->h_cand_all);
    if (e->comm_stream) { (void)hipStreamSynchronize(e->comm_stream); (void)hipStreamDestroy(e->comm_stream); }
    if (e->x_send) (void)hipHostFree(e->x_send);
    if (e->x_recv) (void)hipHostFree(e->x_recv);
    if (e->h_slots) (void)hipHostFree(e->h_slots);
    for (auto &s : e->stage) {
        if (s.nodes) (void)hipHostFree(s.nodes);
        if (s.values) (void)hipHostFree(s.values);
        if (s.arcs) (void)hipHostFree(s.arcs);
        if (s.states) (void)hipHostFree(s.states);
        if (s.done) (void)hipEventDestroy(s.done);
    }
    for (int i = 0; i < mcf_engine::kEvRing; ++i) {
        if (e->ev_start[i]) (void)hipEventDestroy(e->ev_start[i]);
        if (e->ev_stop[i]) (void)hipEventDestroy(e->ev_stop[i]);
    }
    if (e->stream) (void)hipStreamDestroy(e->stream);
    delete e;
}

int mcf_engine_upload(mcf_engine *e, const int32_t *source, const int32_t *target, const int64_t *cost, const int8_t *state, const int64_t *pi)
{
    if (!e || !source || !target || !cost || !state || !pi) return mcf::fail(MCF_ERR_INVALID, "mcf_engine_upload: null argument");
    HIP_TRY(hipSetDevice(e->d.device));
    if (int rcs = resident_stop(e)) return rcs;
    const int n = e->d.node_count, count = e->end - e->begin, cp = e->count_padded;
    for (int i = e->begin; i < e->end; ++i)
        if ((unsigned)source[i] >= (unsigned)n || (unsigned)target[i] >= (unsigned)n)
            return mcf::fail(MCF_ERR_INVALID, "arc %d has an end point outside [0, %d)", i, n);
    int64_t maxc = 0;
    for (int i = e->begin; i < e->end; ++i) maxc = std::max<int64_t>(maxc, cost[i] < 0 ? -cost[i] : cost[i]);
    e->max_abs_cost = maxc;
    std::vector<int32_t> s(cp, 0), t(cp, 0);
    std::vector<int8_t> st(cp, 0);
    const int32_t *pos = nullptr;
    if (e->bucket_nodes > 0) {
        const int buckets = (n + e->bucket_nodes - 1) / e->bucket_nodes;
        std::vector<int32_t> start(buckets + 1, 0);
        for (int i = 0; i < count; ++i) start[target[e->begin + i] / e->bucket_nodes + 1]++;
        for (int b = 0; b < buckets; ++b) start[b + 1] += start[b];
        e->pos_of.resize(count);
        std::vector<int32_t> orig(cp, 0x7FFFFFFF);
        for (int i = 0; i < count; ++i) {
            const int q = start[target[e->begin + i] / e->bucket_nodes]++;
            e->pos_of[i] = q;
            orig[q] = e->begin + i;
        }
        pos = e->pos_of.data();
        HIP_TRY(hipMemcpy(e->d_orig, orig.data(), sizeof(int32_t) * cp, hipMemcpyHostToDevice));
    }
    auto at = [&](int i) { return pos ? pos[i] : i; };
    for (int i = 0; i < count; ++i) { const int q = at(i); s[q] = source[e->begin + i]; t[q] = target[e->begin + i]; st[q] = state[e->begin + i]; }
    HIP_TRY(hipStreamSynchronize(e->stream));
    HIP_TRY(hipMemcpy(e->d_src, s.data(), sizeof(int32_t) * cp, hipMemcpyHostToDevice));
    HIP_TRY(hipMemcpy(e->d_tgt, t.data(), sizeof(int32_t) * cp, hipMemcpyHostToDevice));
    HIP_TRY(hipMemcpy(e->d_state, st.data(), cp, hipMemcpyHostToDevice));
    if (e->d.int_width == 32) {
        std::vector<int32_t> c(cp, 0), p(n);
        for (int i = 0; i < count; ++i) {
            if (!fits32(cost[e->begin + i])) return mcf::fail(MCF_ERR_OVERFLOW, "cost of arc %d does not fit int32", e->begin + i);
            c[at(i)] = (int32_t)cost[e->begin + i];
        }
        for (int i = 0; i < n; ++i) {
            if (!fits32(pi[i])) return mcf::fail(MCF_ERR_OVERFLOW, "potential of node %d does not fit int32", i);
            p[i] = (int32_t)pi[i];
// ... 675 lines not shown
int mcf_engine_park(mcf_engine *e)
{
    if (!e) return mcf::fail(MCF_ERR_INVALID, "null argument");
    (void)hipSetDevice(e->d.device);
    return resident_stop(e);
}

int mcf_engine_get_next_arc(mcf_engine *e, int32_t *next_arc) { if (!e || !next_arc) return mcf::fail(MCF_ERR_INVALID, "null argument"); *next_arc = e->next_arc; return MCF_OK; }
int mcf_engine_set_next_arc(mcf_engine *e, int32_t next_arc)
{
    if (!e || next_arc < 0 || next_arc > e->d.search_arc_num) return mcf::fail(MCF_ERR_INVALID, "next_arc out of range");
    e->next_arc = next_arc;
    return MCF_OK;
}
int mcf_engine_get_block_size(mcf_engine *e, int32_t *b) { if (!e || !b) return mcf::fail(MCF_ERR_INVALID, "null argument"); *b = e->block_size; return MCF_OK; }

int mcf_engine_set_block_config(mcf_engine *e, const mcf_block_config *c, int32_t graph_node_count)
{
    if (!e || !c || graph_node_count < 0) return mcf::fail(MCF_ERR_INVALID, "mcf_engine_set_block_config: bad arguments");
    if (e->st.searches > 0 || e->in_flight != mcf_engine::kNoSearch) return mcf::fail(MCF_ERR_STATE, "mcf_engine_set_block_config: call before the first search");
    if (c->consecutive_hits_before_adapt < 0 || c->min_block_size < 0) return mcf::fail(MCF_ERR_INVALID, "mcf_engine_set_block_config: negative sizes");
    e->cfg = *c;
    e->cfg_set = true;
    e->low_hits = e->high_hits = 0;
    if (e->d.rule != MCF_RULE_BLOCK_SEARCH || e->d.semantics == MCF_SEM_OPTIMIZED) return MCF_OK;
    int32_t b = 0, dyn_min = 0;
    const int rc = mcf_block_initial_size(c, e->d.search_arc_num, graph_node_count, &b, &dyn_min);
    if (rc) return rc;
    e->dyn_min_block = dyn_min;
    if (e->d.block_size <= 0) e->block_size = std::max(1, b);
    e->st.initial_block_size = e->st.current_block_size = e->block_size;
    return MCF_OK;
}

int mcf_engine_download_pi(mcf_engine *e, int64_t *out)
{
    if (!e || !out) return mcf::fail(MCF_ERR_INVALID, "null argument");
    HIP_TRY(hipSetDevice(e->d.device));
    int rc = resident_stop(e);
    if (!rc) rc = flush_pending(e);
    if (rc) return rc;
    HIP_TRY(hipStreamSynchronize(e->stream));
    const int n = e->d.node_count;
    if (e->d.int_width == 32) {
        std::vector<int32_t> t(n);
        HIP_TRY(hipMemcpy(t.data(), e->d_pi, sizeof(int32_t) * n, hipMemcpyDeviceToHost));
        for (int i = 0; i < n; ++i) out[i] = t[i];
    } else {
        HIP_TRY(hipMemcpy(out, e->d_pi, sizeof(int64_t) * n, hipMemcpyDeviceToHost));
    }
    return MCF_OK;
}

int mcf_engine_download_state(mcf_engine *e, int8_t *out)
{
    if (!e || !out) return mcf::fail(MCF_ERR_INVALID, "null argument");
    HIP_TRY(hipSetDevice(e->d.device));
    int rc = resident_stop(e);
    if (!rc) rc = flush_pending(e);
    if (rc) return rc;
    HIP_TRY(hipStreamSynchronize(e->stream));
    if (e->bucket_nodes > 0) {
        std::vector<int8_t> stored(e->end - e->begin);
        HIP_TRY(hipMemcpy(stored.data(), e->d_state, stored.size(), hipMemcpyDeviceToHost));
        for (int i = 0; i < e->end - e->begin; ++i) out[e->begin + i] = stored[e->pos_of[i]];
        return MCF_OK;
    }
    HIP_TRY(hipMemcpy(out + e->begin, e->d_state, e->end - e->begin, hipMemcpyDeviceToHost));
    return MCF_OK;
}

int mcf_engine_get_stats(mcf_engine *e, mcf_engine_stats *out)
{
    if (!e || !out) return mcf::fail(MCF_ERR_INVALID, "null argument");
    (void)hipSetDevice(e->d.device);
    int rc = resident_stop(e);
    if (!rc) rc = drain_events(e, true);
    if (rc) return rc;
    const double ns_per_tick = (mcf::now_ns() - e->cal_ns) / std::max(1.0, (double)__rdtsc() - e->cal_ticks);
    e->st.host_wait_ns = e->wait_ticks * ns_per_tick;
    e->st.host_launch_ns = e->launch_ticks * ns_per_tick;
    e->st.current_block_size = e->block_size;
    e->st.heap_compactions = e->n_heap_sweeps;
    *out = e->st;
    return MCF_OK;
}

int mcf_engine_reset_stats(mcf_engine *e)
{
    if (!e) return mcf::fail(MCF_ERR_INVALID, "null argument");
    (void)hipSetDevice(e->d.device);
    drain_events(e, true);
    const mcf_engine_stats keep = e->st;
    e->st = mcf_engine_stats{};
    e->wait_ticks = e->launch_ticks = 0;
    e->n_heap_sweeps = 0;
    e->st.scan_workgroups = keep.scan_workgroups;
    e->st.scan_threads = keep.scan_threads;
    e->st.bytes_per_scan = keep.bytes_per_scan;
    e->st.resident = keep.resident;
    e->st.candidates = keep.candidates;
    e->st.initial_block_size = keep.initial_block_size;
    e->st.current_block_size = e->block_size;
    e->st.comm_ranks = keep.comm_ranks;
    e->st.scan_bytes_read = keep.scan_bytes_read;
    e->st.rc_layout = keep.rc_layout;
    e->st.shift_grid = keep.shift_grid;
    return MCF_OK;
}

int mcf_engine_bench_scan(mcf_engine *e, int32_t reps, int32_t cold, int64_t flush_bytes, double *avg_ns, double *min_ns)
{
    if (!e || reps < 1 || !avg_ns || !min_ns) return mcf::fail(MCF_ERR_INVALID, "mcf_engine_bench_scan: bad arguments");
    if (e->list_rule) return mcf::fail(MCF_ERR_STATE, "engines of the list rules (3, 4) are searched with mcf_engine_collect_eligible only");
    if (!e->uploaded) return mcf::fail(MCF_ERR_STATE, "mcf_engine_upload has not been called");
    HIP_TRY(hipSetDevice(e->d.device));
    int rc = resident_stop(e);
    if (!rc) rc = flush_pending(e);
    if (rc) return rc;
    if (cold) {
        const size_t want = (size_t)std::max<int64_t>(flush_bytes, 1 << 20);
        if (e->flush_bytes < want) {
            (void)hipFree(e->d_flush);
            e->d_flush = nullptr;
            HIP_TRY(hipMalloc(&e->d_flush, want));
            HIP_TRY(hipMemset(e->d_flush, 0, want));
            e->flush_bytes = want;
        }
    }
    hipEvent_t a, b;
    HIP_TRY(hipEventCreate(&a));
    HIP_TRY(hipEventCreate(&b));
    double sum = 0, mn = 1e30;
    for (int r = 0; r < reps; ++r) {
        if (cold) hipLaunchKernelGGL(flush_kernel, dim3(2048), dim3(256), 0, e->stream, (uint4 *)e->d_flush, e->flush_bytes / 16);
        next_request(e);
        dispatch_search(e, false, a, b);
        HIP_TRY(hipGetLastError());
        HIP_TRY(hipEventSynchronize(b));
        float ms = 0.f;
        HIP_TRY(hipEventElapsedTime(&ms, a, b));
        sum += ms * 1e6;
        mn = std::min(mn, (double)ms * 1e6);
    }
    HIP_TRY(hipStreamSynchronize(e->stream));
    (void)hipEventDestroy(a);
    (void)hipEventDestroy(b);
    *avg_ns = sum / reps;
    *min_ns = mn;
    return MCF_OK;
}

int mcf_engine_bench_update(mcf_engine *e, int32_t count, int32_t reps, double *avg_ns, double *min_ns, int64_t *bytes)
{
    if (!e || count < 1 || count > e->d.node_count || reps < 1 || !avg_ns || !min_ns) return mcf::fail(MCF_ERR_INVALID, "mcf_engine_bench_update: bad arguments");
    if (!e->uploaded) return mcf::fail(MCF_ERR_STATE, "mcf_engine_upload has not been called");
    HIP_TRY(hipSetDevice(e->d.device));
    int rc = resident_stop(e);
    if (!rc) rc = flush_pending(e);
    if (rc) return rc;
    HIP_TRY(hipStreamSynchronize(e->stream));
    const int n = e->d.node_count;
    std::vector<int64_t> cur((size_t)n);
    rc = mcf_engine_download_pi(e, cur.data());
    if (rc) return rc;
    std::vector<int32_t> nodes((size_t)count);
    const int64_t stride = std::max<int64_t>(1, n / count);
    for (int i = 0; i < count; ++i) nodes[i] = (int32_t)((i * stride) % n);
    std::sort(nodes.begin(), nodes.end());
    nodes.erase(std::unique(nodes.begin(), nodes.end()), nodes.end());
    const int k = (int)nodes.size();
    int32_t *d_nodes = nullptr; int64_t *d_vals[2] = {nullptr, nullptr};
    HIP_TRY(hipMalloc((void **)&d_nodes, sizeof(int32_t) * k));
    HIP_TRY(hipMalloc((void **)&d_vals[0], sizeof(int64_t) * k));
    HIP_TRY(hipMalloc((void **)&d_vals[1], sizeof(int64_t) * k));
    std::vector<int64_t> v0((size_t)k), v1((size_t)k);
    int64_t degree = 0;
    for (int i = 0; i < k; ++i) {
        v0[i] = cur[nodes[i]]; v1[i] = cur[nodes[i]] + (e->d.int_width == 32 && cur[nodes[i]] == INT32_MAX ? -1 : 1);
// ... 181 lines not shown
```

### mincostflow_amd/csrc/kernels.hip.h

```cpp
#pragma once

#include <hip/hip_runtime.h>

#include <cstdint>

#include "../../include/mcf_hip.h"
#include "mailbox.hip.h"

namespace {


constexpr int kThreads = 256;
constexpr int kArcsPerThread = 4;
constexpr int kTile = kThreads * kArcsPerThread;
constexpr int kPad = 8 * kTile;
constexpr int kInlinePi = 96;
constexpr int kInlineState = 4;
constexpr int kMaxWorkgroups = 8192;
constexpr uint32_t kNone = 0xFFFFFFFFu;
constexpr int kSlotStride = 4;
constexpr int kResidentThreads = 1024;
constexpr int kResidentTile = kResidentThreads * kArcsPerThread;
constexpr int kLdsPiMax = 16384;

// ... 503 lines not shown
    out.x = (uint32_t)(uint64_t)c;
    out.y = (uint32_t)((uint64_t)c >> 32);
    out.z = p;
    out.w = record_tag(tag, c, p);
    asm volatile("global_store_dwordx4 %0, %1, off sc0 sc1" ::"v"(slot), "v"(out) : "memory");
}

constexpr int kCandPerGroup = 3;
constexpr int kCandRecords = 4;

template <typename T>
__device__ __forceinline__ void fold_tile_best2(const TileData<T> &d, const T ps[4], const T pt[4], int e0, int64_t &c1, uint32_t &p1, int64_t &c2, uint32_t &p2)
{
    c1 = 0; p1 = kNone; c2 = 0; p2 = kNone;
#pragma unroll
    for (int j = 0; j < 4; ++j) {
        const int st = (int)(int8_t)(d.st4 >> (8 * j));
        const int64_t dd = (int64_t)d.c.v[j] + (int64_t)ps[j] - (int64_t)pt[j];
        const int64_t rc = st > 0 ? dd : (st < 0 ? -dd : 0);
        const uint32_t e = (uint32_t)(e0 + j);
        const bool b1 = rc < c1;
        const bool b2 = !b1 && rc < c2;
        c2 = b1 ? c1 : (b2 ? rc : c2);
        p2 = b1 ? p1 : (b2 ? e : p2);
        c1 = b1 ? rc : c1;
        p1 = b1 ? e : p1;
    }
}

template <typename T>
__device__ __forceinline__ void eval_tile_best2(const TileData<T> &d, const T *pi, int e0, int64_t &c1, uint32_t &p1, int64_t &c2, uint32_t &p2,
                                                int sub_node, T sub_val)
{
    T ps[4], pt[4];
#pragma unroll
    for (int j = 0; j < 4; ++j) { ps[j] = pi[d.s.v[j]]; pt[j] = pi[d.t.v[j]]; }
#pragma unroll
    for (int j = 0; j < 4; ++j) { ps[j] = d.s.v[j] == sub_node ? sub_val : ps[j]; pt[j] = d.t.v[j] == sub_node ? sub_val : pt[j]; }
    fold_tile_best2<T>(d, ps, pt, e0, c1, p1, c2, p2);
}

__device__ __forceinline__ void publish_candidates(int64_t c1, uint32_t p1, int64_t c2, uint32_t p2, Slot *slots, uint32_t tag)
{
    const int tid = threadIdx.x;
    __shared__ Cand wave_first[kResidentThreads / 64], wave_second[kResidentThreads / 64];
    int64_t wc = c1;
    uint32_t wp = p1;
    cand_wave_min(wc, wp);
    int64_t sc = (p1 == wp && p1 != kNone) ? c2 : c1;
    uint32_t sp = (p1 == wp && p1 != kNone) ? p2 : p1;
    cand_wave_min(sc, sp);
    if ((tid & 63) == 0) { wave_first[tid >> 6] = Cand{wc, wp}; wave_second[tid >> 6] = Cand{sc, sp}; }
    __syncthreads();
    if (tid < 64) {
        const int waves = (int)(blockDim.x >> 6);
        int64_t fc = 0, tc = 0;
        uint32_t fp = kNone, tp = kNone;
        if (tid < waves) { fc = wave_first[tid].c; fp = wave_first[tid].p; tc = wave_second[tid].c; tp = wave_second[tid].p; }
        int64_t kc[kCandPerGroup];
        uint32_t kp[kCandPerGroup];
#pragma unroll
        for (int k = 0; k < kCandPerGroup; ++k) {
            int64_t mc = fc;
            uint32_t mp = fp;
            cand_wave_min(mc, mp);
            kc[k] = mc;
            kp[k] = mp;
            const bool mine = mp != kNone && fp == mp;
            fc = mine ? 0 : fc;
            fp = mine ? kNone : fp;
        }
        if (cand_less(fc, fp, tc, tp)) { tc = fc; tp = fp; }
        cand_wave_min(tc, tp);
        if (tid < kCandRecords) {
            int64_t oc = tc;
            uint32_t op = tp;
#pragma unroll
            for (int k = 0; k < kCandPerGroup; ++k) { oc = tid == k ? kc[k] : oc; op = tid == k ? kp[k] : op; }
            store_record_system(slots + (size_t)blockIdx.x * kCandRecords + tid, oc, op, tag);
        }
    }
}

constexpr int kPiRegCompare = 20;
constexpr int kPiRegBitmapMax = 4096;
constexpr int kPiRegBitmapWords = 4096;

constexpr int kPiRegThreads = 512;

template <typename T, int RULE, bool OPT, bool REG, bool LPI, bool CAND, bool PIREG = false, bool PERM = false>
__global__ __launch_bounds__(PIREG ? kPiRegThreads : kResidentThreads) void resident_kernel(const ResidentParams<T> p)
{
    static_assert(!PERM || (RULE == MCF_RULE_BEST_ELIGIBLE && !REG && !LPI && !CAND), "the bucketed layout serves the tile loop of Best Eligible");
    static_assert(!PIREG || (REG && !LPI), "PIREG needs register-resident arcs and global potentials");
    constexpr int kLines = LPI ? kMailboxLines : 2 * kMailboxLines, kChunk = kLines - 1;
    __shared__ __attribute__((aligned(16))) uint32_t lm[kLines * 16];
    __shared__ __attribute__((aligned(16))) T lpi[LPI ? kLdsPiMax : 2];
    __shared__ uint32_t s_timeout;
    __shared__ uint32_t bitmap[PIREG ? kPiRegBitmapWords : 1];
    const int tid = threadIdx.x, nt = (int)blockDim.x;
    const int my_i0 = blockIdx.x * nt * kArcsPerThread + tid * kArcsPerThread;
    TileData<T> mine;
    if (REG) load_tile<T>(p.src, p.tgt, p.cost, p.state, my_i0, mine);
    T ps[4], pt[4];
    if (PIREG) {
        gather_tile<T>(mine, p.pi, ps, pt);
        for (int i = tid; i < kPiRegBitmapWords; i += nt) bitmap[i] = 0u;
        __syncthreads();
    }
    if (LPI) {
        for (int i = tid; i < p.n_nodes; i += nt) lpi[i] = p.pi[i];
        __syncthreads();
    }
    const T *const pi_view = LPI ? lpi : p.pi;
    uint32_t last = p.mb.start_seq, served = 0, last_sub = 0;
    int applied = 0;
    uint64_t scan_ticks = 0;
    uint64_t idle_since = __builtin_amdgcn_s_memrealtime();
    const uint32_t *const my_unit = p.mb.mailbox + (size_t)(blockIdx.x % p.mb.poll_replicas) * kReplicaStride;
    for (;;) {
        const bool timed_out = poll_request<kHdrApplySub>(my_unit, last, last_sub, [](uint32_t c) { return c == kCmdApply; }, idle_since, p.mb, lm, s_timeout);
        const uint32_t seq = lm[kHdrSeq];
        const int n_pi = clamp_count((int)lm[kHdrValues], p.mb.max_pi), n_st = clamp_count((int)lm[kHdrStates], p.mb.max_st);
        const int extra_pi = n_pi > 1 ? n_pi - 1 : 0, extra_st = n_st > 2 ? n_st - 2 : 0;
        const int entries = extra_pi + extra_st;
        const uint32_t cmd = lm[kHdrCmd];
        const bool apply_only = cmd == kCmdApply;
        const uint32_t sub = lm[kHdrApplySub];
        const int upto = clamp_count((int)lm[kHdrApplyLines], (p.mb.max_pi + p.mb.max_st) / kMailboxPatchesPerLine);
        const int lines = apply_only ? upto : (entries + kMailboxPatchesPerLine - 1) / kMailboxPatchesPerLine;
        const bool line1_staged = lm[16 + 15] == seq;
        const int next_arc = (int)lm[kHdrNextArc], rstar = (int)lm[kHdrRstar];
        const int block_size = (int)lm[kHdrBlockSize] > 0 ? (int)lm[kHdrBlockSize] : 1;
        const int st_arc0 = (int)lm[kHdrState0], st_arc1 = (int)lm[kHdrState0 + 2];
        const uint32_t st_val0 = lm[kHdrState0 + 1], st_val1 = lm[kHdrState0 + 3];
        const uint32_t p0_node = lm[kHdrValue0], p0_lo = lm[kHdrValue0 + 1], p0_hi = lm[kHdrValue0 + 2];
        if (lines > 0) __syncthreads();
        if (timed_out || cmd == kCmdQuit) {
            if (tid == 0 && blockIdx.x == 0) resident_exit(p.mb.exit_word, timed_out ? kExitIdle : kExitQuit, served, scan_ticks);
            return;
        }
        const uint64_t t_seen = blockIdx.x == 0 ? __builtin_amdgcn_s_memrealtime() : 0;
        const int pr_mode = !PIREG ? 0 : ((apply_only || applied > 0) ? 3 : (entries == 0 ? 0 : (entries <= kPiRegCompare ? 1 : (entries <= kPiRegBitmapMax ? 2 : 3))));
        const int entries_here = apply_only ? upto * kMailboxPatchesPerLine : entries;
        const int pi_here = apply_only ? entries_here : extra_pi;
        bool torn = false;
        for (int first = applied; first < lines; first += kChunk) {
            const int chunk = lines - first < kChunk ? lines - first : kChunk;
            const bool staged = first == 0 && chunk == 1 && line1_staged;
            if (!stage_lines<4>(lm + 16, p.mb.mailbox, my_unit, 0, 0, 0, staged ? 0 : chunk, first, seq)) { torn = true; break; }
            const int i_lo = first * kMailboxPatchesPerLine;
            const int i_hi = entries_here < i_lo + chunk * kMailboxPatchesPerLine ? entries_here : i_lo + chunk * kMailboxPatchesPerLine;
            for (int i = i_lo + tid; i < i_hi; i += nt) {
                const int rel = i - i_lo;
                const uint32_t *q = entry_at(lm + 16, rel);
                if (i < pi_here) {
                    const int64_t v = (int64_t)(((uint64_t)q[2] << 32) | q[1]);
                    p.pi[q[0]] = (T)v;
                    if (LPI) lpi[q[0]] = (T)v;
                    if (pr_mode == 2) atomicOr(&bitmap[(q[0] >> 5) & (kPiRegBitmapWords - 1)], 1u << (q[0] & 31));
                } else {
                    const int a = (int)q[0] - p.base;
                    if ((unsigned)a < (unsigned)p.count_padded) p.state[a] = (int8_t)q[1];
                }
            }
            if (pr_mode == 1) {
// ... 29 lines not shown
        const bool fast = REG && (entries == 0 || pr_mode == 1) && applied == 0;
        const T v0 = (T)(int64_t)(((uint64_t)p0_hi << 32) | p0_lo);
        if (n_pi | n_st) {
            if (tid == 0 && n_pi > 0) { p.pi[p0_node] = v0; if (LPI) lpi[p0_node] = v0; }
            if (tid == 1 && n_st > 0) { const int a = st_arc0 - p.base; if ((unsigned)a < (unsigned)p.count_padded) p.state[a] = (int8_t)st_val0; }
            if (tid == 2 && n_st > 1) { const int a = st_arc1 - p.base; if ((unsigned)a < (unsigned)p.count_padded) p.state[a] = (int8_t)st_val1; }
            if (REG) {
                if (n_st > 0) { const int a = st_arc0 - p.base - my_i0; if ((unsigned)a < 4u) mine.st4 = (mine.st4 & ~(0xFFu << (8 * a))) | ((st_val0 & 0xFFu) << (8 * a)); }
                if (n_st > 1) { const int a = st_arc1 - p.base - my_i0; if ((unsigned)a < 4u) mine.st4 = (mine.st4 & ~(0xFFu << (8 * a))) | ((st_val1 & 0xFFu) << (8 * a)); }
            }
            if (!fast) {
                __builtin_amdgcn_s_waitcnt(0);
                __syncthreads();
            }
        }
        const int sub_node = (fast && n_pi > 0) ? (int)p0_node : -1;
        if (PIREG) {
            if (pr_mode == 2) {
#pragma unroll
                for (int j = 0; j < 4; ++j) {
                    const uint32_t a = (uint32_t)mine.s.v[j], b = (uint32_t)mine.t.v[j];
                    if ((bitmap[(a >> 5) & (kPiRegBitmapWords - 1)] >> (a & 31)) & 1u) ps[j] = p.pi[a];
                    if ((bitmap[(b >> 5) & (kPiRegBitmapWords - 1)] >> (b & 31)) & 1u) pt[j] = p.pi[b];
                }
                __syncthreads();
                for (int i = tid; i < kPiRegBitmapWords; i += nt) bitmap[i] = 0u;
            } else if (pr_mode == 3) {
                gather_tile<T>(mine, p.pi, ps, pt);
            }
            if (n_pi > 0) {
#pragma unroll
                for (int j = 0; j < 4; ++j) { ps[j] = mine.s.v[j] == (int)p0_node ? v0 : ps[j]; pt[j] = mine.t.v[j] == (int)p0_node ? v0 : pt[j]; }
            }
        }
        if (CAND) {
            int64_t c1, c2;
            uint32_t p1, p2;
            if (PIREG) fold_tile_best2<T>(mine, ps, pt, p.base + my_i0, c1, p1, c2, p2);
            else eval_tile_best2<T>(mine, pi_view, p.base + my_i0, c1, p1, c2, p2, sub_node, v0);
            publish_candidates(c1, p1, c2, p2, p.slots, seq);
        } else {
            Key best{0, kNone, kNone}, range{0, kNone, kNone};
            if (PIREG) {
                fold_tile<T, RULE, OPT>(mine, ps, pt, p.base + my_i0, p.m_s, next_arc, block_size, rstar, best, range);
            } else if (REG) {
                eval_tile<T, RULE, OPT>(mine, pi_view, p.base + my_i0, p.m_s, next_arc, block_size, rstar, best, range, sub_node, v0);
            } else {
                for (int i0 = my_i0; i0 < p.count_padded; i0 += gridDim.x * nt * kArcsPerThread) {
                    TileData<T> d;
                    load_tile<T>(p.src, p.tgt, p.cost, p.state, i0, d);
                    eval_tile<T, RULE, OPT, PERM>(d, pi_view, p.base + i0, p.m_s, next_arc, block_size, rstar, best, range, -1, (T)0, p.orig, p.base);
                }
                if (PERM && best.p != kNone) best.p = (uint32_t)p.orig[(int)best.p - p.base];
            }
            publish_best<RULE, true, kResidentThreads, kDual<RULE, OPT>>(best, p.slots + (size_t)blockIdx.x * kSlotStride, seq, true, range);
        }
        last = seq;
        applied = 0;
        served += 1;
        idle_since = __builtin_amdgcn_s_memrealtime();
        if (blockIdx.x == 0) scan_ticks += idle_since - t_seen;
        if (fast) __builtin_amdgcn_s_waitcnt(0);
        __syncthreads();
    }
}

constexpr int kShiftBits = 131072;
constexpr int kCandLines = 512;
constexpr int kCandRoundLines = 480;
constexpr int kCandHash = 4096;
constexpr uint32_t kHashEmpty = 0xFFFFFFFFu;
constexpr int kCandCompare = 3;

constexpr int kCandThreads = 256;
template <typename T, int TILES>
__global__ __launch_bounds__(kCandThreads) void resident_cand_kernel(const ResidentParams<T> p, const uint32_t shift_base, const int max_shift_lines)
{
    __shared__ __attribute__((aligned(16))) uint32_t lm[kCandLines * 16];
    __shared__ uint32_t bitmap[kShiftBits / 32];
    __shared__ uint32_t vmap[kShiftBits / 32];
    __shared__ uint32_t hkey[kCandHash];
    __shared__ __attribute__((aligned(8))) int64_t hval[kCandHash];
    __shared__ uint32_t s_timeout;
    __shared__ uint32_t sp_mask[TILES * kCandThreads], sp_val[TILES * kCandThreads];
    const int tid = threadIdx.x, nt = (int)blockDim.x;
    int my_i[TILES];
    TileData<T> mine[TILES];
    T ps[TILES][4], pt[TILES][4];
#pragma unroll
    for (int t = 0; t < TILES; ++t) {
        my_i[t] = (t * (int)gridDim.x + (int)blockIdx.x) * nt * kArcsPerThread + tid * kArcsPerThread;
        const int at = my_i[t] < p.count_padded ? my_i[t] : 0;
        load_tile<T>(p.src, p.tgt, p.cost, p.state, at, mine[t]);
        if (my_i[t] >= p.count_padded) mine[t].st4 = 0u;
        gather_tile<T>(mine[t], p.pi, ps[t], pt[t]);
    }
    for (int i = tid; i < kShiftBits / 32; i += nt) { bitmap[i] = 0u; vmap[i] = 0u; }
    for (int i = tid; i < kCandHash; i += nt) hkey[i] = kHashEmpty;
    for (int i = tid; i < TILES * kCandThreads; i += nt) { sp_mask[i] = 0u; sp_val[i] = 0u; }
    __syncthreads();
    auto post_state = [&](int arc, uint32_t val) {
        const int local = arc - p.base;
        if ((unsigned)local >= (unsigned)p.count_padded) return;
        const int tile = local / (nt * kArcsPerThread), t = tile / (int)gridDim.x;
        if (tile % (int)gridDim.x != (int)blockIdx.x || t >= TILES) return;
        const int r = local % (nt * kArcsPerThread), owner = r / kArcsPerThread, slot = r % kArcsPerThread;
        atomicOr(&sp_mask[t * kCandThreads + owner], 0xFFu << (8 * slot));
        atomicOr(&sp_val[t * kCandThreads + owner], (val & 0xFFu) << (8 * slot));
    };
    uint32_t last = p.mb.start_seq, served = 0, last_sub = 0, shifted_for = p.mb.start_seq;
    int shift_done = 0;
    bool bits_set = false;
    uint32_t reloaded_for = p.mb.start_seq, barriers = 0;
    uint64_t scan_ticks = 0;
    uint64_t ph_shift = 0, ph_values = 0, ph_scan = 0, n_shift_req = 0;
    const uint64_t born_rt = __builtin_amdgcn_s_memrealtime(), born_clk = __builtin_amdgcn_s_memtime();
    uint64_t idle_since = __builtin_amdgcn_s_memrealtime();
    const uint32_t *const my_unit = p.mb.mailbox + (size_t)(blockIdx.x % p.mb.poll_replicas) * kReplicaStride;
    constexpr int kStage = 32;
    constexpr int kChunk = kCandLines - 2;
    auto fetch = [&](int n_a, int first_a, int n_v, int first_v, uint32_t seq) -> bool {
        return stage_lines<4>(lm + kStage, p.mb.mailbox, my_unit, shift_base, n_a, first_a, n_v, first_v, seq);
    };
    for (;;) {
        const bool timed_out = poll_request<kShHdrApplySub>(my_unit, last, last_sub, [](uint32_t c) { return c == kCmdApply || c == kCmdApplyRuns; },
                                                            idle_since, p.mb, lm, s_timeout);
        const uint32_t seq = lm[kHdrSeq], cmd = lm[kHdrCmd], sub = lm[kShHdrApplySub];
        const int n_val = clamp_count((int)lm[kShHdrValues], p.mb.max_pi), n_st = clamp_count((int)lm[kHdrStates], p.mb.max_st);
        const bool apply_only = cmd == kCmdApply || cmd == kCmdApplyRuns;
        const bool ranges = apply_only ? cmd == kCmdApplyRuns : lm[kShHdrRuns] == 1u;
        const int per_line = ranges ? kShiftPairsPerLine : kShiftNodesPerLine;
        const int n_shift = apply_only ? 0 : clamp_count((int)lm[kShHdrShift], max_shift_lines * per_line);
        const int shift_lines = clamp_count(apply_only ? (int)lm[kShHdrShift] : (n_shift + per_line - 1) / per_line, max_shift_lines);
        const int64_t sigma = (int64_t)(((uint64_t)lm[kShHdrSigma + 1] << 32) | lm[kShHdrSigma]);
        const bool line1_staged = lm[16 + 15] == seq;
        const int st_arc0 = (int)lm[kHdrState0], st_arc1 = (int)lm[kHdrState0 + 2];
        const uint32_t st_val0 = lm[kHdrState0 + 1], st_val1 = lm[kHdrState0 + 3];
        const uint32_t v0_node = lm[kHdrValue0];
        const T v0 = (T)(int64_t)(((uint64_t)lm[kHdrValue0 + 2] << 32) | lm[kHdrValue0 + 1]);
        if (timed_out || cmd == kCmdQuit) {
            if (tid == 0 && blockIdx.x == 0) {
                const uint64_t d_rt = __builtin_amdgcn_s_memrealtime() - born_rt, d_clk = __builtin_amdgcn_s_memtime() - born_clk;
                n_shift_req = d_rt ? d_clk * 100 / d_rt : 0;
                const uint64_t ph[4] = {ph_shift, ph_values, ph_scan, n_shift_req};
                for (int q = 0; q < 4; ++q) {
                    __hip_atomic_store(p.mb.exit_word + 4 + 2 * q, (uint32_t)ph[q], __ATOMIC_RELAXED, __HIP_MEMORY_SCOPE_SYSTEM);
                    __hip_atomic_store(p.mb.exit_word + 5 + 2 * q, (uint32_t)(ph[q] >> 32), __ATOMIC_RELAXED, __HIP_MEMORY_SCOPE_SYSTEM);
                }
                resident_exit(p.mb.exit_word, timed_out ? kExitIdle : kExitQuit, served, scan_ticks);
            }
            return;
        }
        const uint64_t t_seen = blockIdx.x == 0 ? __builtin_amdgcn_s_memrealtime() : 0;
        if (cmd == kCmdReload && p.mb.host_pi && reloaded_for != seq) {
            reload_slice(p.pi, sizeof(T) == 4, p.mb.host_pi, p.n_nodes);
            if (!grid_barrier(p.mb, barriers, s_timeout)) {
                if (tid == 0) resident_exit(p.mb.exit_word, kExitBarrier, served, scan_ticks);
                return;
            }
#pragma unroll
            for (int t = 0; t < TILES; ++t) gather_tile<T>(mine[t], p.pi, ps[t], pt[t]);
            if (bits_set) {
                for (int i = tid; i < kShiftBits / 32; i += nt) bitmap[i] = 0u;
                bits_set = false;
                __syncthreads();
            }
            shift_done = 0;
            reloaded_for = seq;
        }
        const int extra_val = n_val > 1 ? n_val - 1 : 0, extra_st = n_st > 2 ? n_st - 2 : 0, entries = apply_only ? 0 : extra_val + extra_st;
        const int lines = (entries + kMailboxPatchesPerLine - 1) / kMailboxPatchesPerLine;
        const bool inline_entries = lines == 1 && line1_staged;
        const int need_v = inline_entries ? 0 : lines;
        auto set_bits = [&](int off, int first, int chunk) {
            if (ranges) {
                const int left = n_shift - first * kShiftPairsPerLine;
                const int pairs_here = apply_only ? chunk * kShiftPairsPerLine : (left < chunk * kShiftPairsPerLine ? left : chunk * kShiftPairsPerLine);
                for (int i = tid; i < pairs_here; i += nt) {
                    const uint32_t *q = lm + kStage + (off + i / kShiftPairsPerLine) * 16 + 2 * (i % kShiftPairsPerLine);
                    const uint32_t a = q[0];
                    uint32_t len = q[1];
                    if (a >= (uint32_t)kShiftBits || len == 0u) continue;
                    if (len > (uint32_t)kShiftBits - a) len = (uint32_t)kShiftBits - a;
                    const uint32_t z = a + len - 1u;
                    for (uint32_t w = a >> 5; w <= (z >> 5); ++w) {
                        uint32_t mask = 0xFFFFFFFFu;
                        if (w == (a >> 5)) mask &= 0xFFFFFFFFu << (a & 31u);
                        if (w == (z >> 5)) mask &= 0xFFFFFFFFu >> (31u - (z & 31u));
                        atomicOr(&bitmap[w], mask);
                    }
                }
                return;
            }
            const int left = n_shift - first * kShiftNodesPerLine;
            const int nodes_here = apply_only ? chunk * kShiftNodesPerLine : (left < chunk * kShiftNodesPerLine ? left : chunk * kShiftNodesPerLine);
            int p2 = 64;
            while (p2 < nodes_here) p2 <<= 1;
            for (int x = tid; x < p2; x += nt) {
                const int i = (x * 37) & (p2 - 1);
                if (i < nodes_here) {
                    const uint32_t u = lm[kStage + (off + i / kShiftNodesPerLine) * 16 + i % kShiftNodesPerLine];
                    if (u < (uint32_t)kShiftBits) atomicOr(&bitmap[u >> 5], 1u << (u & 31));
                }
            }
        };
        auto shift_once = [&]() {
            if (n_shift > 0 && shifted_for != seq) {
                uint32_t wa[TILES][4], wb[TILES][4];
#pragma unroll
                for (int t = 0; t < TILES; ++t)
#pragma unroll
                    for (int j = 0; j < 4; ++j) {
                        wa[t][j] = bitmap[((uint32_t)mine[t].s.v[j] >> 5) & (kShiftBits / 32 - 1)];
// ... 69 lines not shown
#pragma unroll
                    for (int j = 0; j < 8; ++j) {
                        const uint32_t node = (uint32_t)(j < 4 ? mine[t].s.v[j & 3] : mine[t].t.v[j & 3]);
                        if ((marks >> (8 * t + j)) & 1u) {
                            uint32_t h = (node * 2654435761u) >> 20;
                            for (int step = 0; step < kCandHash; ++step) {
                                const uint32_t k = hkey[h];
                                if (k == kHashEmpty) break;
                                if (k == node) { const T v = (T)hval[h]; if (j < 4) ps[t][j & 3] = v; else pt[t][j & 3] = v; break; }
                                h = (h + 1) & (kCandHash - 1);
                            }
                        }
                    }
                __syncthreads();
                for (int i = i_lo + tid; i < v_hi; i += nt) {
                    const int rel = i - i_lo;
                    const uint32_t node = *entry_at(at, rel);
                    vmap[(node >> 5) & (kShiftBits / 32 - 1)] = 0u;
                }
                for (int i = tid; i < kCandHash; i += nt) hkey[i] = kHashEmpty;
            }
            if (extra_st > 0 && i_hi > extra_val) {
                const int s_lo = i_lo > extra_val ? i_lo : extra_val;
                for (int i = s_lo + tid; i < i_hi; i += nt) {
                    const int rel = i - i_lo;
                    const uint32_t *q = entry_at(at, rel);
                    post_state((int)q[0], q[1]);
                }
            }
        };
        bool torn = false;
        uint64_t t_shifted = 0;
        const int pend_a = shift_lines - shift_done;
        if (!apply_only && pend_a + need_v <= kChunk && need_v <= kCandRoundLines) {
            if (pend_a + need_v > 0) {
                if (!fetch(pend_a, shift_done, need_v, 0, seq)) continue;
                if (pend_a > 0) { set_bits(0, shift_done, pend_a); bits_set = true; shift_done += pend_a; __syncthreads(); }
            }
            t_shifted = blockIdx.x == 0 ? __builtin_amdgcn_s_memrealtime() : 0;
            shift_once();
            if (inline_entries) apply_entries(lm + 16, 0, 1);
            else if (need_v > 0) apply_entries(lm + kStage + pend_a * 16, 0, need_v);
        } else {
            for (int first = shift_done; first < shift_lines; first += kChunk) {
                const int chunk = shift_lines - first < kChunk ? shift_lines - first : kChunk;
                if (!fetch(chunk, first, 0, 0, seq)) { torn = true; break; }
                set_bits(0, first, chunk);
                bits_set = true;
                shift_done = first + chunk;
                __syncthreads();
            }
            if (torn) continue;
            if (apply_only) {
                last_sub = sub;
                idle_since = __builtin_amdgcn_s_memrealtime();
                continue;
            }
            t_shifted = blockIdx.x == 0 ? __builtin_amdgcn_s_memrealtime() : 0;
            shift_once();
            if (inline_entries) apply_entries(lm + 16, 0, 1);
            else {
                for (int first = 0; first < lines; first += kCandRoundLines) {
                    const int chunk = lines - first < kCandRoundLines ? lines - first : kCandRoundLines;
                    if (!fetch(0, 0, chunk, first, seq)) { torn = true; break; }
                    apply_entries(lm + kStage, first, chunk);
                    __syncthreads();
                }
                if (torn) continue;
            }
        }
        if (n_st > 0) {
            __syncthreads();
#pragma unroll
            for (int t = 0; t < TILES; ++t) {
                const uint32_t m = sp_mask[t * kCandThreads + tid];
                if (m) {
                    mine[t].st4 = (mine[t].st4 & ~m) | (sp_val[t * kCandThreads + tid] & m);
                    sp_mask[t * kCandThreads + tid] = 0u;
                    sp_val[t * kCandThreads + tid] = 0u;
                }
            }
        }
        const uint64_t t_patched = blockIdx.x == 0 ? __builtin_amdgcn_s_memrealtime() : 0;
        int64_t c1 = 0, c2 = 0;
        uint32_t p1 = kNone, p2 = kNone;
#pragma unroll
        for (int t = 0; t < TILES; ++t)
#pragma unroll
            for (int j = 0; j < 4; ++j) {
                const int st = (int)(int8_t)(mine[t].st4 >> (8 * j));
                const int64_t dd = (int64_t)mine[t].c.v[j] + (int64_t)ps[t][j] - (int64_t)pt[t][j];
                const int64_t rc = st > 0 ? dd : (st < 0 ? -dd : 0);
                const uint32_t e = (uint32_t)(p.base + my_i[t] + j);
                const bool b1 = rc < c1;
                const bool b2 = !b1 && rc < c2;
                c2 = b1 ? c1 : (b2 ? rc : c2);
                p2 = b1 ? p1 : (b2 ? e : p2);
                c1 = b1 ? rc : c1;
                p1 = b1 ? e : p1;
            }
        publish_candidates(c1, p1, c2, p2, p.slots, seq);
        if (bits_set) {
            for (int i = tid; i < kShiftBits / 32; i += nt) bitmap[i] = 0u;
            bits_set = false;
        }
        shift_done = 0;
        last = seq;
        served += 1;
        idle_since = __builtin_amdgcn_s_memrealtime();
        if (blockIdx.x == 0) {
            scan_ticks += idle_since - t_seen;
            ph_shift += t_shifted - t_seen; ph_values += t_patched - t_shifted; ph_scan += idle_since - t_patched;
            n_shift_req += n_shift > 0 ? 1 : 0;
        }
        __syncthreads();
    }
}

constexpr int kRcWindow = 8192;
constexpr int kRcResidentNodes = 1 + 255 * kMailboxPatchesPerLine - 8;

__device__ __forceinline__ void fold_rc_best2(uint32_t st4, const int64_t d[4], int e0, int64_t &c1, uint32_t &p1, int64_t &c2, uint32_t &p2)
{
#pragma unroll
    for (int j = 0; j < 4; ++j) {
        const int st = (int)(int8_t)(st4 >> (8 * j));
        const int64_t rc = st > 0 ? d[j] : (st < 0 ? -d[j] : 0);
        const uint32_t e = (uint32_t)(e0 + j);
        const bool b1 = rc < c1;
        const bool b2 = !b1 && rc < c2;
        c2 = b1 ? c1 : (b2 ? rc : c2);
        p2 = b1 ? p1 : (b2 ? e : p2);
        c1 = b1 ? rc : c1;
        p1 = b1 ? e : p1;
    }
}

struct ResidentRcParams {
    int8_t *state;
    int64_t *rc;
    void *pi;
    const int32_t *adj_start;
    const uint32_t *adj;
    Slot *slots;
    const int32_t *src, *tgt;
    const void *cost;
    int32_t base, count_padded, m_s, window;
    int32_t narrow, n_nodes;
    MailboxParams mb;
};

template <int RULE, bool OPT, bool LD, bool CAND = false>
__global__ __launch_bounds__(kResidentThreads) void resident_rc_kernel(const ResidentRcParams p)
{
    static_assert(!CAND || RULE == MCF_RULE_BEST_ELIGIBLE, "candidate lists serve Best Eligible");
    constexpr int kLines = kMailboxLines;
    constexpr int kChunk = kLines - 1;
    constexpr int kNodesMax = 1280;
    __shared__ __attribute__((aligned(16))) uint32_t lm[kLines * 16];
    __shared__ __attribute__((aligned(16))) int64_t ld[LD ? kRcWindow : 2];
    __shared__ __attribute__((aligned(16))) int8_t ls[LD ? kRcWindow : 4];
    __shared__ int32_t s_node[kNodesMax], s_lo[kNodesMax], s_pre[kNodesMax + 1];
    __shared__ int64_t s_delta[kNodesMax];
    __shared__ uint32_t s_timeout;
    const int tid = threadIdx.x, nt = (int)blockDim.x;
    const int w_lo = LD ? (int)blockIdx.x * p.window : 0;
    typedef long v2l __attribute__((ext_vector_type(2)));
    auto load_window = [&]() {
        for (int i = tid * 4; i < p.window; i += nt * 4) {
            const int g = w_lo + i;
            if (g < p.count_padded) {
                *reinterpret_cast<v2l *>(ld + i) = *reinterpret_cast<const v2l *>(p.rc + g);
                *reinterpret_cast<v2l *>(ld + i + 2) = *reinterpret_cast<const v2l *>(p.rc + g + 2);
                *reinterpret_cast<uint32_t *>(ls + i) = *reinterpret_cast<const uint32_t *>(p.state + g);
            } else {
                ld[i] = ld[i + 1] = ld[i + 2] = ld[i + 3] = 0;
                *reinterpret_cast<uint32_t *>(ls + i) = 0u;
            }
        }
        __syncthreads();
    };
    if (LD) load_window();
    uint32_t last = p.mb.start_seq, served = 0, prog_seq = p.mb.start_seq, barriers = 0;
    int prog_lines = 0;
// ... 318 lines not shown
```

### mincostflow_amd/csrc/mailbox.hip.h

```cpp
#pragma once

#include <hip/hip_runtime.h>
#include <immintrin.h>

#include <cstdint>
#include <cstring>

namespace {

constexpr int kMailboxLines = 256;
constexpr int kMailboxPatchesPerLine = 5;
constexpr int kMaxReplicas = 16;
constexpr int kReplicaStride = 1024;
constexpr int kMailboxTail = kMaxReplicas * kReplicaStride;
constexpr int kShiftNodesPerLine = 15;
constexpr int kShiftPairsPerLine = 7;

enum : uint32_t {
    kCmdScan = 0,
    kCmdQuit = 1,
    kCmdApply = 2,
    kCmdReload = 3,
    kCmdApplyRuns = 4,
};
enum : uint32_t {
    kExitQuit = 1,
    kExitIdle = 2,
    kExitBarrier = 3,
    kExitPartial = 4,
};
enum : int {
    kHdrSeq = 0, kHdrCmd = 1,
    kHdrStates = 5,
    kHdrState0 = 6,
    kHdrValue0 = 10,
    kHdrTag = 15,
    kHdrNextArc = 2, kHdrRstar = 3,
    kHdrValues = 4,
    kHdrBlockSize = 13,
    kHdrApplyLines = 13,
    kHdrApplySub = 14,
    kShHdrValues = 2,
    kShHdrShift = 3,
    kShHdrRuns = 4,
    kShHdrApplySub = 4,
    kShHdrSigma = 13,
};

struct MailboxParams {
    const uint32_t *mailbox;
    uint32_t *exit_word;
    uint32_t start_seq, idle_ticks;
    int32_t max_pi;
    int32_t max_st;
    int32_t poll_replicas, poll_sleep;
    const int64_t *host_pi;
    uint32_t *barrier;
};

typedef uint32_t v4u __attribute__((ext_vector_type(4)));

__device__ __forceinline__ int clamp_count(int x, int hi) { return x < 0 ? 0 : (x > hi ? hi : x); }

__device__ __forceinline__ const uint32_t *entry_line(const uint32_t *mailbox, const uint32_t *unit, int l)
{
    return l == 0 ? unit + 16 : mailbox + (kMailboxTail + (size_t)(l - 1) * 16);
}
__device__ __forceinline__ const uint32_t *entry_at(const uint32_t *base, int i)
{
    return base + (i / kMailboxPatchesPerLine) * 16 + 3 * (i % kMailboxPatchesPerLine);
}

template <int SUB_WORD, typename IsApply>
__device__ __forceinline__ bool poll_request(const uint32_t *unit, uint32_t last, uint32_t last_sub, IsApply is_apply, uint64_t idle_since,
                                             const MailboxParams &mb, uint32_t *lm, uint32_t &s_flag)
{
    const int tid = threadIdx.x;
    if (tid < 64) {
        v4u x = v4u{0u, 0u, 0u, 0u};
        uint32_t flag;
        for (;;) {
            if (tid < 8) asm volatile("global_load_dwordx4 %0, %1, off sc0 sc1" : "=v"(x) : "v"(unit + tid * 4) : "memory");
            asm volatile("s_waitcnt vmcnt(0)" : "+v"(x)::"memory");
            const uint32_t seq0 = (uint32_t)__builtin_amdgcn_readlane((int)x[0], 0), tag0 = (uint32_t)__builtin_amdgcn_readlane((int)x[3], 3);
            bool fresh = seq0 != last && tag0 == seq0;
            if constexpr (SUB_WORD >= 0) {
                const uint32_t cmd0 = (uint32_t)__builtin_amdgcn_readlane((int)x[1], 0), sub0 = (uint32_t)__builtin_amdgcn_readlane((int)x[SUB_WORD & 3], SUB_WORD >> 2);
                fresh = fresh && (!is_apply(cmd0) || sub0 != last_sub);
            }
            if (fresh) { flag = 1u; break; }
            if (__builtin_amdgcn_s_memrealtime() - idle_since > mb.idle_ticks) { flag = kExitIdle; break; }
            for (int z = 0; z < mb.poll_sleep; ++z) __builtin_amdgcn_s_sleep(1);
        }
        if (tid < 8) *reinterpret_cast<v4u *>(lm + tid * 4) = x;
        if (tid == 0) s_flag = flag;
    }
    __syncthreads();
    return s_flag == kExitIdle;
}

template <int DEPTH>
__device__ __forceinline__ bool stage_lines(uint32_t *dst, const uint32_t *mailbox, const uint32_t *unit, uint32_t shift_base, int n_a, int first_a,
                                            int n_v, int first_v, uint32_t seq)
{
    static_assert(DEPTH == 1 || DEPTH == 4, "one or four reads per wait");
    const int tid = threadIdx.x, nt = (int)blockDim.x;
    const int count = n_a + n_v;
    for (int base = 0; base < count * 4; base += nt * DEPTH) {
        v4u x[DEPTH];
#pragma unroll
        for (int q = 0; q < DEPTH; ++q) {
            x[q] = v4u{0u, 0u, 0u, 0u};
            const int c = base + q * nt + tid;
            if (c < count * 4) {
                const int l = c >> 2;
                const uint32_t *src = l < n_a ? mailbox + (shift_base + (size_t)(first_a + l) * 16) : entry_line(mailbox, unit, first_v + l - n_a);
                asm volatile("global_load_dwordx4 %0, %1, off sc0 sc1" : "=v"(x[q]) : "v"(src + (c & 3) * 4) : "memory");
            }
        }
        if constexpr (DEPTH == 4) asm volatile("s_waitcnt vmcnt(0)" : "+v"(x[0]), "+v"(x[1]), "+v"(x[2]), "+v"(x[3])::"memory");
        else asm volatile("s_waitcnt vmcnt(0)" : "+v"(x[0])::"memory");
#pragma unroll
        for (int q = 0; q < DEPTH; ++q) {
            const int c = base + q * nt + tid;
            if (c < count * 4) *reinterpret_cast<v4u *>(dst + c * 4) = x[q];
        }
    }
    __syncthreads();
    int bad = 0;
// ... 116 lines not shown
```

### mincostflow_amd/network_simplex.py

```python
from __future__ import annotations

import ctypes as C
from dataclasses import dataclass

import numpy as np

from . import _lib as L
from ._lib import McfError


class PivotRule:
    FirstEligible, BestEligible, BlockSearch, CandidateList, AlteringList = 0, 1, 2, 3, 4


class SupplyType:
    Geq, Leq = 0, 1


class SolverStatus:
    NotSolved, Optimal, Infeasible, Unbounded, Unbalanced = 0, 1, 2, 3, 4


class Verdict:
    NoVerdict, Feasible, Cut, Open, Bounds = L.DIAG_NONE, L.DIAG_FEASIBLE, L.DIAG_CUT, L.DIAG_OPEN, L.DIAG_BOUNDS
# ... 1033 lines not shown
        return v.value

    def reload_potentials(self, changed_nodes: int):
        L.check(L.lib().mcf_engine_reload_potentials(self._h, changed_nodes))

    def renumber_nodes(self, new_of):
        new_of = _i32(new_of)
        assert new_of.shape == (self.node_count,)
        L.check(L.lib().mcf_engine_renumber_nodes(self._h, new_of))

    def check_reduced_costs(self):
        m, f = C.c_int64(), C.c_int32()
        L.check(L.lib().mcf_engine_check_reduced_costs(self._h, C.byref(m), C.byref(f)))
        return m.value, f.value

    def patch_arcs(self, arcs, source, target, cost):
        arcs = _i32(arcs)
        L.check(L.lib().mcf_engine_patch_arcs(self._h, len(arcs), arcs, _i32(source), _i32(target), _i64(cost)))

    def find_entering(self):
        f, a, c = C.c_int32(), C.c_int32(), C.c_int64()
        L.check(L.lib().mcf_engine_find_entering(self._h, C.byref(f), C.byref(a), C.byref(c)))
        return bool(f.value), a.value, c.value

    def search_begin(self):
        L.check(L.lib().mcf_engine_search_begin(self._h))

    def search_end(self):
        f, a, c = C.c_int32(), C.c_int32(), C.c_int64()
        L.check(L.lib().mcf_engine_search_end(self._h, C.byref(f), C.byref(a), C.byref(c)))
        return bool(f.value), a.value, c.value

    def search_end_local(self) -> L.Candidate:
        c = L.Candidate()
        L.check(L.lib().mcf_engine_search_end_local(self._h, C.byref(c)))
        return c

    def find_entering_local(self) -> L.Candidate:
        c = L.Candidate()
        L.check(L.lib().mcf_engine_find_entering_local(self._h, C.byref(c)))
        return c

    def resolve(self, cands):
        arr = (L.Candidate * len(cands))(*cands)
        f, a, c = C.c_int32(), C.c_int32(), C.c_int64()
        L.check(L.lib().mcf_engine_resolve(self._h, len(cands), arr, C.byref(f), C.byref(a), C.byref(c)))
        return bool(f.value), a.value, c.value

    def collect_eligible(self, next_arc: int, *, limit: int = 0, block_size: int = 0, head_length: int = 0, survivors: int = 0, capacity: int = None):
        mode = L.COLLECT_FIRST_N if limit > 0 else L.COLLECT_BLOCKS
        if capacity is None:
            capacity = limit if mode == L.COLLECT_FIRST_N else head_length + block_size
        rq = L.CollectRequest(next_arc, mode, limit, block_size, head_length, survivors)
        arcs, rcs = np.zeros(max(capacity, 1), np.int32), np.zeros(max(capacity, 1), np.int64)
        k, end, scanned = C.c_int32(), C.c_int32(), C.c_int64()
        L.check(L.lib().mcf_engine_collect_eligible(self._h, C.byref(rq), capacity, C.byref(k), arcs.ctypes.data, rcs.ctypes.data,
                                                    C.byref(end), C.byref(scanned)))
        return arcs[: k.value].copy(), rcs[: k.value].copy(), end.value, scanned.value

    @property
    def next_arc(self) -> int:
        v = C.c_int32(); L.check(L.lib().mcf_engine_get_next_arc(self._h, C.byref(v))); return v.value

    @next_arc.setter
    def next_arc(self, v: int):
        L.check(L.lib().mcf_engine_set_next_arc(self._h, v))

    @property
    def block_size(self) -> int:
        v = C.c_int32(); L.check(L.lib().mcf_engine_get_block_size(self._h, C.byref(v))); return v.value

    def set_block_config(self, config, graph_node_count: int):
        L.check(L.lib().mcf_engine_set_block_config(self._h, C.byref(config), graph_node_count))

    def download_pi(self) -> np.ndarray:
        out = np.empty(self.node_count, np.int64); L.check(L.lib().mcf_engine_download_pi(self._h, out)); return out

    def download_state(self) -> np.ndarray:
        out = np.zeros(self.arc_capacity, np.int8); L.check(L.lib().mcf_engine_download_state(self._h, out)); return out

    def stats(self) -> dict:
        s = L.EngineStats(); L.check(L.lib().mcf_engine_get_stats(self._h, C.byref(s))); return s.as_dict()

    def park(self):
        L.check(L.lib().mcf_engine_park(self._h))

    def reset_stats(self):
        L.check(L.lib().mcf_engine_reset_stats(self._h))

    def bench_scan(self, reps=20, cold=False, flush_bytes=512 << 20):
        avg, mn = C.c_double(), C.c_double()
        L.check(L.lib().mcf_engine_bench_scan(self._h, reps, int(cold), flush_bytes, C.byref(avg), C.byref(mn)))
        return avg.value, mn.value


class HostExchange:

    def __init__(self, name: str, rank: int, world: int):
        self.world = world
        self._h = C.c_void_p()
        L.check(L.lib().mcf_exchange_open(C.byref(self._h), name.encode(), rank, world))

    def all_gather(self, mine: "L.Candidate"):
        out = (L.Candidate * self.world)()
        L.check(L.lib().mcf_exchange_all_gather(self._h, C.byref(mine), out))
        return list(out)

    def close(self):
        if self._h:
            L.lib().mcf_exchange_close(self._h)
            self._h = None

    def __del__(self):
        self.close()


def _bench_update(self, count, reps=20):
    avg, mn, nb = C.c_double(), C.c_double(), C.c_int64()
    L.check(L.lib().mcf_engine_bench_update(self._h, count, reps, C.byref(avg), C.byref(mn), C.byref(nb)))
    return avg.value, mn.value, nb.value


PivotEngine.bench_update = _bench_update


def _bench_search(self, reps=1000):
    avg, mn = C.c_double(), C.c_double()
    L.check(L.lib().mcf_engine_bench_search(self._h, reps, C.byref(avg), C.byref(mn)))
    return avg.value, mn.value


PivotEngine.bench_search = _bench_search


def shard_range(search_arc_num: int, rank: int, world: int):
    b, e = C.c_int32(), C.c_int32()
    L.check(L.lib().mcf_shard_range(search_arc_num, rank, world, C.byref(b), C.byref(e)))
    return b.value, e.value


def resolve_candidates(rule: int, optimized: bool, search_arc_num: int, block_size: int, next_arc: int, cands, vector_width=4):
    arr = (L.Candidate * len(cands))(*cands)
    na, f, a, c = C.c_int32(next_arc), C.c_int32(), C.c_int32(), C.c_int64()
    L.check(L.lib().mcf_resolve_candidates(rule, L.SEM_OPTIMIZED if optimized else L.SEM_PLAIN, _vector_width_abi(vector_width), search_arc_num, block_size,
                                           C.byref(na), len(cands), arr, C.byref(f), C.byref(a), C.byref(c)))
    return bool(f.value), a.value, c.value, na.value
```

Before: 304,200.

## Return bounded per-workgroup candidate lists from resident shift-grid scan

The resident shift-grid scan can now take an adaptive reduced-cost bound. Each workgroup lists every arc below that bound, up to a fixed cap, instead of reporting only its top two, and the host installs these richer candidate lists. The bound gap is learned from each installed list, narrowing when lists overflow and widening when they come back short, so more candidates are gathered per device round trip and fewer scans are needed. The cost is an extra ballot pass and a shared-memory atomic in the kernel, more slot records to poll on the host, and a change to the mailbox header encoding.

```diff
diff --git a/include/mcf_hip.h b/include/mcf_hip.h
--- a/include/mcf_hip.h
+++ b/include/mcf_hip.h
@@ -191,9 +191,19 @@
     int64_t shift_lists;
     int64_t mirror_uploads;
     double phase_shift_ns, phase_values_ns, phase_scan_ns;
+    int64_t lists_installed;
+    int64_t list_entries;
+    int64_t group_overflows;
+    int64_t bound_widenings;
+    int64_t bound_narrowings;
 } mcf_engine_stats;
 MCF_API int mcf_engine_get_stats(mcf_engine *e, mcf_engine_stats *out);
 MCF_API int mcf_engine_reset_stats(mcf_engine *e);
+
+enum { MCF_CAND_BOUND_AUTO = 0, MCF_CAND_BOUND_NONE = 1, MCF_CAND_BOUND_FIXED = 2 };
+MCF_API int mcf_engine_candidate_list_control(mcf_engine *e, int32_t mode, int64_t bound, int32_t target);
+MCF_API int mcf_engine_candidate_list(mcf_engine *e, int32_t capacity, uint32_t *arcs, int64_t *keys, int32_t *count, int64_t *thr_key,
+                                      uint32_t *thr_arc, uint32_t *epoch);
 
 MCF_API int mcf_engine_bench_scan(mcf_engine *e, int32_t reps, int32_t cold, int64_t flush_bytes,
                                   double *avg_ns, double *min_ns);
diff --git a/mincostflow_amd/_lib.py b/mincostflow_amd/_lib.py
--- a/mincostflow_amd/_lib.py
+++ b/mincostflow_amd/_lib.py
@@ -54,7 +54,9 @@
                 ("resident_requests", C.c_int64), ("resident_scan_ns", C.c_double), ("resident_kernel_ns", C.c_double), ("candidates", C.c_int64),
                 ("host_decided", C.c_int64), ("arcs_checked", C.c_int64), ("initial_block_size", C.c_int32), ("current_block_size", C.c_int32),
                 ("comm_ranks", C.c_int32), ("reserved", C.c_int32), ("async_refreshes", C.c_int64), ("scan_bytes_read", C.c_int64), ("rc_layout", C.c_int64), ("rc_recomputes", C.c_int64), ("renumberings", C.c_int64), ("heap_compactions", C.c_int64), ("rc_reloads_in_grid", C.c_int64), ("shift_grid", C.c_int64), ("shift_lists", C.c_int64), ("mirror_uploads", C.c_int64),
-                ("phase_shift_ns", C.c_double), ("phase_values_ns", C.c_double), ("phase_scan_ns", C.c_double)]
+                ("phase_shift_ns", C.c_double), ("phase_values_ns", C.c_double), ("phase_scan_ns", C.c_double),
+                ("lists_installed", C.c_int64), ("list_entries", C.c_int64), ("group_overflows", C.c_int64), ("bound_widenings", C.c_int64),
+                ("bound_narrowings", C.c_int64)]
 
     def as_dict(self):
         return {n: getattr(self, n) for n, _ in self._fields_ if n != "reserved"}
@@ -340,6 +342,9 @@
     "mcf_engine_download_pi": (C.c_int, [C.c_void_p, _i64p]),
     "mcf_engine_download_state": (C.c_int, [C.c_void_p, _i8p]),
     "mcf_engine_get_stats": (C.c_int, [C.c_void_p, _P(EngineStats)]),
+    "mcf_engine_candidate_list_control": (C.c_int, [C.c_void_p, C.c_int32, C.c_int64, C.c_int32]),
+    "mcf_engine_candidate_list": (C.c_int, [C.c_void_p, C.c_int32, np.ctypeslib.ndpointer(np.uint32, flags="C_CONTIGUOUS"), _i64p, _P(C.c_int32), _P(C.c_int64),
+                                  _P(C.c_uint32), _P(C.c_uint32)]),
     "mcf_engine_reset_stats": (C.c_int, [C.c_void_p]),
     "mcf_engine_bench_scan": (C.c_int, [C.c_void_p, C.c_int32, C.c_int32, C.c_int64, _P(C.c_double), _P(C.c_double)]),
     "mcf_engine_bench_search": (C.c_int, [C.c_void_p, C.c_int32, _P(C.c_double), _P(C.c_double)]),
diff --git a/mincostflow_amd/csrc/candidate_cache.hip.h b/mincostflow_amd/csrc/candidate_cache.hip.h
--- a/mincostflow_amd/csrc/candidate_cache.hip.h
+++ b/mincostflow_amd/csrc/candidate_cache.hip.h
@@ -132,10 +132,18 @@
     return MCF_OK;
 }
 
+inline int cand_stride(const mcf_engine *e) { return e->shift_grid ? kListRecords : kCandRecords; }
+inline bool cand_slot_ready(const volatile Slot &r, uint32_t seq) { const int64_t c = r.c; const uint32_t q = r.p; return r.tag == record_tag(seq, c, q); }
+
 bool cand_records_ready(const mcf_engine *e, int g)
 {
-    const volatile Slot *rec = e->h_slots + (size_t)g * kCandRecords;
-    for (int r = 0; r < kCandRecords; ++r) { const int64_t c = rec[r].c; const uint32_t q = rec[r].p; if (rec[r].tag != record_tag(e->seq, c, q)) return false; }
+    const volatile Slot *rec = e->h_slots + (size_t)g * cand_stride(e);
+    for (int r = 0; r < kCandRecords; ++r) if (!cand_slot_ready(rec[r], e->seq)) return false;
+    if (!e->shift_grid) return true;
+    const int64_t extras = rec[kListHead - 1].c;
+    if (extras < 0 || extras > kListHits) return false;
+    const int records = (kListHead + (int)extras + 3) & ~3;
+    for (int r = kCandRecords; r < records; ++r) if (!cand_slot_ready(rec[r], e->seq)) return false;
     return true;
 }
 
@@ -146,8 +154,10 @@
     const volatile Slot *slots = e->h_slots;
     e->cand_records.clear();
     mcf_engine::CandKey thr{0, kNone};
+    const int stride = cand_stride(e);
+    int overflowed = 0;
     for (int g = 0; g < e->res_grid; ++g) {
-        const volatile Slot *rec = slots + (size_t)g * kCandRecords;
+        const volatile Slot *rec = slots + (size_t)g * stride;
         uint64_t spins = 0;
         while (!cand_records_ready(e, g)) {
             _mm_pause();
@@ -169,15 +179,26 @@
             }
         }
         std::atomic_thread_fence(std::memory_order_acquire);
-        for (int r = 0; r < kCandPerGroup; ++r)
-            if (rec[r].p != kNone) e->cand_records.push_back(mcf_engine::CandKey{rec[r].c, rec[r].p});
-        if (rec[kCandPerGroup].p != kNone) {
-            const mcf_engine::CandKey t{rec[kCandPerGroup].c, rec[kCandPerGroup].p};
+        int thr_at = kCandPerGroup;
+        if (e->shift_grid) {
+            thr_at = 1;
+            if (rec[0].p != kNone) e->cand_records.push_back(mcf_engine::CandKey{rec[0].c, rec[0].p});
+            const int extras = (int)rec[kListHead - 1].c;
+            for (int r = kListHead; r < kListHead + extras; ++r)
+                if (rec[r].p != kNone) e->cand_records.push_back(mcf_engine::CandKey{rec[r].c, rec[r].p});
+            if (rec[kListHead - 1].p & kListOverflow) overflowed += 1;
+        } else {
+            for (int r = 0; r < kCandPerGroup; ++r)
+                if (rec[r].p != kNone) e->cand_records.push_back(mcf_engine::CandKey{rec[r].c, rec[r].p});
+        }
+        if (rec[thr_at].p != kNone) {
+            const mcf_engine::CandKey t{rec[thr_at].c, rec[thr_at].p};
             if (thr.p == kNone || cand_key_less(t, thr)) thr = t;
         }
     }
     e->wait_ticks += (double)__rdtsc() - t0;
-    cand_install(e, cand_graph(e), e->cand_records.data(), e->cand_records.size(), thr, at);
+    cand_install(e, cand_graph(e), e->cand_records.data(), e->cand_records.size(), thr, at, overflowed, e->shift_grid && e->req_bounded);
+    if (e->cand_debug) e->list_lengths.push_back((int32_t)e->cand_list.size());
     e->tk_collect += (double)__rdtsc() - t0;
     return MCF_OK;
 }
@@ -268,9 +289,12 @@
         e->shift_streamed = 0;
     }
     MailboxLine h = request_header(e, seq, cmd, n_st, n_val, val_lo);
+    const bool with_bound = (cmd == kCmdScan || cmd == kCmdReload) && e->req_bounded;
+    h.w[kHdrCmd] = cmd | (with_patches && runs ? kShCmdRuns : 0u) | (with_bound ? kShCmdBound : 0u) | ((uint32_t)n_st << kShCmdStatesShift);
     h.w[kShHdrValues] = (uint32_t)n_val;
     h.w[kShHdrShift] = with_patches ? (uint32_t)n_shift : 0u;
-    h.w[kShHdrRuns] = with_patches && runs ? 1u : 0u;
+    h.w[kShHdrBound] = with_bound ? (uint32_t)(uint64_t)e->req_bound : 0u;
+    h.w[kShHdrBound + 1] = with_bound ? (uint32_t)((uint64_t)e->req_bound >> 32) : 0u;
     h.w[kShHdrSigma] = (uint32_t)(uint64_t)sigma;
     h.w[kShHdrSigma + 1] = (uint32_t)((uint64_t)sigma >> 32);
     mailbox_publish(e->mailbox, kPollReplicas, h, vals.n + sts.n > 0 ? &line1 : nullptr);
@@ -297,6 +321,13 @@
     e->stream_lines = complete;
 }
 
+inline void cand_choose_bound(mcf_engine *e)
+{
+    if (e->bound_mode == MCF_CAND_BOUND_NONE) e->req_bounded = false;
+    else if (e->bound_mode == MCF_CAND_BOUND_FIXED) { e->req_bounded = true; e->req_bound = e->bound_fixed; }
+    else e->req_bounded = cand_bound_next(e, &e->req_bound);
+}
+
 int cand_post_shift(mcf_engine *e)
 {
     if (!e->resident_running) {
@@ -318,6 +349,7 @@
         e->pend_state.resize(e->pend_arc.size());
         for (size_t i = 0; i < e->pend_arc.size(); ++i) e->pend_state[i] = e->h_state[e->pend_arc[i]];
         next_request_keep_prev(e);
+        cand_choose_bound(e);
         shift_post_request(e, e->seq, kCmdReload, 0, 0, 0, true);
         e->st.rc_reloads_in_grid += 1;
         e->pend_arc.clear(); e->pend_state.clear();
@@ -353,6 +385,7 @@
         e->pend_state.resize(e->pend_arc.size());
         for (size_t i = 0; i < e->pend_arc.size(); ++i) e->pend_state[i] = e->h_state[e->pend_arc[i]];
         next_request_keep_prev(e);
+        cand_choose_bound(e);
         shift_post_request(e, e->seq, kCmdScan, val_lo, as_shift ? (runs ? n_pairs : n_b) : 0, e->pend_sigma, true, runs);
         if (!e->pend_node.empty() || !e->pend_arc.empty()) e->st.inline_updates += 1;
         if (as_shift) e->st.shift_lists += 1;
diff --git a/mincostflow_amd/csrc/candidate_state.h b/mincostflow_amd/csrc/candidate_state.h
--- a/mincostflow_amd/csrc/candidate_state.h
+++ b/mincostflow_amd/csrc/candidate_state.h
@@ -9,6 +9,7 @@
 constexpr uint32_t kCandNone = 0xFFFFFFFFu;
 constexpr int kCandMaxNodes = 256;
 constexpr int64_t kCandDegreePerNode = 8;
+constexpr int kCandListTarget = 48;
 
 struct CandState {
     struct AdjEnt { int32_t arc; uint32_t other; int64_t cost; };
@@ -35,7 +36,44 @@
     bool async_posted = false;
     size_t heap_compact_above = 1u << 18;
     int64_t n_heap_push = 0, n_heap_admit = 0, n_heap_pop = 0, n_heap_sweeps = 0;
+    bool bound_seeded = false;
+    int64_t bound_gap = 0;
+    int64_t bound_best = 0;
+    int bound_target = kCandListTarget;
+    int64_t n_lists = 0, n_list_entries = 0, n_group_overflows = 0, n_bound_widen = 0, n_bound_narrow = 0;
+    uint32_t list_at = 0;
+    std::vector<CandKey> list_installed;
+    bool keep_installed = false;
 };
+
+inline bool cand_bound_next(const CandState *e, int64_t *x)
+{
+    if (!e->bound_seeded) return false;
+    const int64_t room = -e->bound_best;
+    *x = e->bound_gap >= room ? 0 : e->bound_best + e->bound_gap;
+    return true;
+}
+
+inline void cand_bound_learn(CandState *e, size_t listed, int64_t best_c, CandState::CandKey thr, int overflowed, bool bounded)
+{
+    const int64_t kGapMax = INT64_MAX / 4;
+    if (listed > 0) e->bound_best = best_c;
+    if (!e->bound_seeded) {
+        if (listed == 0 || thr.p == kCandNone) return;
+        e->bound_gap = std::max<int64_t>(1, thr.c - best_c);
+        e->bound_seeded = true;
+        return;
+    }
+    if (!bounded) return;
+    const size_t target = (size_t)std::max(1, e->bound_target);
+    if (overflowed > 0 || listed > 2 * target) {
+        e->bound_gap = std::max<int64_t>(1, e->bound_gap - e->bound_gap / 3);
+        e->n_bound_narrow += 1;
+    } else if (2 * listed < target && thr.p != kCandNone) {
+        e->bound_gap = std::min<int64_t>(kGapMax, e->bound_gap + e->bound_gap / 2 + 1);
+        e->n_bound_widen += 1;
+    }
+}
 
 struct CandGraph {
     const int32_t *adj_start;
@@ -204,11 +242,13 @@
     } else {
         return false;
     }
+    if (win.p != kCandNone) e->bound_best = win.c;
     *out = win;
     return true;
 }
 
-inline void cand_install(CandState *e, const CandGraph &g, const CandState::CandKey *rec, size_t n, CandState::CandKey thr, uint32_t at)
+inline void cand_install(CandState *e, const CandGraph &g, const CandState::CandKey *rec, size_t n, CandState::CandKey thr, uint32_t at,
+                         int overflowed = 0, bool bounded = false)
 {
     e->cand_thr = thr;
     e->cand_list.clear();
@@ -222,6 +262,12 @@
     e->hd_ok = e->tp_ok = false;
     e->snap_at = at;
     e->async_posted = false;
+    e->n_lists += 1;
+    e->n_list_entries += (int64_t)e->cand_list.size();
+    e->n_group_overflows += overflowed;
+    e->list_at = at;
+    if (e->keep_installed) e->list_installed = e->cand_list;
+    cand_bound_learn(e, e->cand_list.size(), e->cand_list.empty() ? 0 : e->cand_list[0].c, thr, overflowed, bounded);
     cand_sweep_heap(e, true);
 }
 
@@ -234,6 +280,9 @@
     e->heap.clear();
     e->pivot_nodes.clear(); e->pivot_arcs.clear(); e->pivot_degree = 0; e->pivot_overflow = false;
     e->heap_gap = e->cand_now;
+    e->bound_seeded = false;
+    e->bound_gap = e->bound_best = 0;
+    e->list_installed.clear();
 }
 
 constexpr uint32_t kCandEpochWrap = 0xFFFFFF00u;
diff --git a/mincostflow_amd/csrc/engine.hip b/mincostflow_amd/csrc/engine.hip
--- a/mincostflow_amd/csrc/engine.hip
+++ b/mincostflow_amd/csrc/engine.hip
@@ -182,6 +182,10 @@
     int64_t call_shift = 0;
     std::vector<CandState::CandKey> cand_records;
     uint32_t async_at = 0, posted_at = 0;
+    bool req_bounded = false;
+    int64_t req_bound = 0, bound_fixed = 0;
+    int32_t bound_mode = MCF_CAND_BOUND_AUTO;
+    std::vector<int32_t> list_lengths;
     int patch_capacity = 0;
     uint32_t cand_epoch0 = 1;
     bool cand_debug = false;
@@ -756,9 +760,10 @@
         chk(hipMalloc((void **)&e->d_adj_start, sizeof(int32_t) * ((size_t)desc->node_count + 1)));
         chk(hipMalloc((void **)&e->d_adj, sizeof(uint32_t) * (size_t)std::max(1, 2 * count)));
     }
-    chk(hipHostMalloc((void **)&e->h_slots, sizeof(Slot) * kMaxWorkgroups * kSlotStride, hipHostMallocMapped | hipHostMallocCoherent));
+    const size_t n_slots = std::max<size_t>((size_t)kMaxWorkgroups * kSlotStride, (size_t)kResidentMaxGrid * kListRecords);
+    chk(hipHostMalloc((void **)&e->h_slots, sizeof(Slot) * n_slots, hipHostMallocMapped | hipHostMallocCoherent));
     if (err == hipSuccess) {
-        memset(e->h_slots, 0, sizeof(Slot) * kMaxWorkgroups * kSlotStride);
+        memset(e->h_slots, 0, sizeof(Slot) * n_slots);
         chk(hipHostGetDevicePointer((void **)&e->d_slots, e->h_slots, 0));
     }
     for (int i = 0; i < 2 && err == hipSuccess; ++i) {
@@ -891,17 +896,27 @@
 }
 }
 
+namespace {
+int list_median(mcf_engine *e)
+{
+    if (e->list_lengths.empty()) return 0;
+    std::nth_element(e->list_lengths.begin(), e->list_lengths.begin() + e->list_lengths.size() / 2, e->list_lengths.end());
+    return e->list_lengths[e->list_lengths.size() / 2];
+}
+}
+
 void mcf_engine_destroy(mcf_engine *e)
 {
     if (!e) return;
     if (e->cand_on && e->cand_debug && e->st.searches > 1000) {
         const double ns_per_tick = (mcf::now_ns() - e->cal_ns) / std::max(1.0, (double)__rdtsc() - e->cal_ticks);
         const double n = (double)e->st.searches;
-        fprintf(stderr, "[cand] searches %lld host %lld async %lld sync_posts %lld async_waits %lld gap_pivots %lld | per search ns: absorb %.0f probe %.0f decide %.0f post %.0f collect %.0f wait %.0f | heap size %zu pushes %lld admitted %lld pops %lld sweeps %lld\n",
+        fprintf(stderr, "[cand] searches %lld host %lld async %lld sync_posts %lld async_waits %lld gap_pivots %lld | per search ns: absorb %.0f probe %.0f decide %.0f post %.0f collect %.0f wait %.0f | heap size %zu pushes %lld admitted %lld pops %lld sweeps %lld | lists %lld entries %lld median %d group_overflows %lld widen %lld narrow %lld\n",
                 (long long)e->st.searches, (long long)e->st.host_decided, (long long)e->st.async_refreshes, (long long)e->n_sync_posts, (long long)e->n_async_waits,
                 (long long)e->n_gap_pivots, e->tk_absorb * ns_per_tick / n, e->tk_probe * ns_per_tick / n, e->tk_decide * ns_per_tick / n, e->tk_post * ns_per_tick / n,
                 e->tk_collect * ns_per_tick / n, e->wait_ticks * ns_per_tick / n, e->heap.size(), (long long)e->n_heap_push, (long long)e->n_heap_admit, (long long)e->n_heap_pop,
-                (long long)e->n_heap_sweeps);
+                (long long)e->n_heap_sweeps, (long long)e->n_lists, (long long)e->n_list_entries, list_median(e), (long long)e->n_group_overflows,
+                (long long)e->n_bound_widen, (long long)e->n_bound_narrow);
     }
     (void)hipSetDevice(e->d.device);
     (void)resident_stop(e);
@@ -1743,7 +1758,37 @@
     e->st.host_launch_ns = e->launch_ticks * ns_per_tick;
     e->st.current_block_size = e->block_size;
     e->st.heap_compactions = e->n_heap_sweeps;
+    e->st.lists_installed = e->n_lists;
+    e->st.list_entries = e->n_list_entries;
+    e->st.group_overflows = e->n_group_overflows;
+    e->st.bound_widenings = e->n_bound_widen;
+    e->st.bound_narrowings = e->n_bound_narrow;
     *out = e->st;
+    return MCF_OK;
+}
+
+int mcf_engine_candidate_list_control(mcf_engine *e, int32_t mode, int64_t bound, int32_t target)
+{
+    if (!e) return mcf::fail(MCF_ERR_INVALID, "null argument");
+    if (mode != MCF_CAND_BOUND_AUTO && mode != MCF_CAND_BOUND_NONE && mode != MCF_CAND_BOUND_FIXED) return mcf::fail(MCF_ERR_INVALID, "mcf_engine_candidate_list_control: unknown mode");
+    if (target < 0) return mcf::fail(MCF_ERR_INVALID, "mcf_engine_candidate_list_control: negative target");
+    e->bound_mode = mode;
+    e->bound_fixed = bound;
+    if (target > 0) e->bound_target = target;
+    e->keep_installed = true;
+    return MCF_OK;
+}
+
+int mcf_engine_candidate_list(mcf_engine *e, int32_t capacity, uint32_t *arcs, int64_t *keys, int32_t *count, int64_t *thr_key, uint32_t *thr_arc, uint32_t *epoch)
+{
+    if (!e || !count || capacity < 0 || (capacity > 0 && (!arcs || !keys))) return mcf::fail(MCF_ERR_INVALID, "mcf_engine_candidate_list: bad arguments");
+    if (!e->cand_on || !e->cand_valid) return mcf::fail(MCF_ERR_STATE, "mcf_engine_candidate_list: no list has been installed");
+    if (!e->keep_installed) return mcf::fail(MCF_ERR_STATE, "mcf_engine_candidate_list: call mcf_engine_candidate_list_control first (the list is only kept when asked for)");
+    *count = (int32_t)e->list_installed.size();
+    for (int32_t i = 0; i < *count && i < capacity; ++i) { arcs[i] = e->list_installed[i].p; keys[i] = e->list_installed[i].c; }
+    if (thr_key) *thr_key = e->cand_thr.c;
+    if (thr_arc) *thr_arc = e->cand_thr.p;
+    if (epoch) *epoch = e->list_at;
     return MCF_OK;
 }
 
@@ -1756,6 +1801,7 @@
     e->st = mcf_engine_stats{};
     e->wait_ticks = e->launch_ticks = 0;
     e->n_heap_sweeps = 0;
+    e->n_lists = e->n_list_entries = e->n_group_overflows = e->n_bound_widen = e->n_bound_narrow = 0;
     e->st.scan_workgroups = keep.scan_workgroups;
     e->st.scan_threads = keep.scan_threads;
     e->st.bytes_per_scan = keep.bytes_per_scan;
diff --git a/mincostflow_amd/csrc/kernels.hip.h b/mincostflow_amd/csrc/kernels.hip.h
--- a/mincostflow_amd/csrc/kernels.hip.h
+++ b/mincostflow_amd/csrc/kernels.hip.h
@@ -609,6 +609,79 @@
     }
 }
 
+constexpr int kListLines = 4;
+constexpr int kListRecords = 4 * kListLines;
+constexpr int kListHead = 3;
+constexpr int kListHits = kListRecords - kListHead;
+constexpr uint32_t kListOverflow = 1u;
+
+__device__ __forceinline__ void publish_list(bool listed, bool bounded, uint32_t hits, int64_t c1, uint32_t p1, int64_t c2, uint32_t p2,
+                                             const Cand *s_hit, uint32_t &s_hits, Slot *slots, uint32_t tag)
+{
+    const int tid = threadIdx.x;
+    __shared__ Cand wave_first[kResidentThreads / 64], wave_second[kResidentThreads / 64];
+    int64_t wc = c1, sc = 0;
+    uint32_t wp = p1, sp = kNone;
+    cand_wave_min(wc, wp);
+    if (!listed) {
+        sc = (p1 == wp && p1 != kNone) ? c2 : c1;
+        sp = (p1 == wp && p1 != kNone) ? p2 : p1;
+        cand_wave_min(sc, sp);
+    }
+    if ((tid & 63) == 0) { wave_first[tid >> 6] = Cand{wc, wp}; wave_second[tid >> 6] = Cand{sc, sp}; }
+    __syncthreads();
+    if (tid == 0) s_hits = 0u;
+    if (tid >= 64) return;
+    const int waves = (int)(blockDim.x >> 6);
+    int64_t fc = 0, tc = 0, oc = 0;
+    uint32_t fp = kNone, tp = kNone, op = kNone, extras = 0, flags = 0;
+    if (tid < waves) { fc = wave_first[tid].c; fp = wave_first[tid].p; tc = wave_second[tid].c; tp = wave_second[tid].p; }
+    if (listed) {
+        cand_wave_min(fc, fp);
+        int64_t hc = 0, bc;
+        uint32_t hp = kNone, bp;
+        if ((uint32_t)tid < hits) { hc = s_hit[tid].c; hp = s_hit[tid].p; }
+        bc = hc; bp = hp;
+        cand_wave_min(bc, bp);
+        const int best_lane = __ffsll((long long)__ballot(hp == bp && hp != kNone)) - 1;
+        extras = hits - 1u;
+        const int k = tid - kListHead;
+        const int src = tid == 0 ? best_lane : (k >= 0 ? (k < best_lane ? k : k + 1) : 0);
+        oc = __shfl(hc, src & 63);
+        op = __shfl(hp, src & 63);
+        if (k >= (int)extras) { oc = 0; op = kNone; }
+        tc = fc; tp = fp;
+    } else {
+        int64_t kc[kCandPerGroup];
+        uint32_t kp[kCandPerGroup];
+#pragma unroll
+        for (int k = 0; k < kCandPerGroup; ++k) {
+            int64_t mc = fc;
+            uint32_t mp = fp;
+            cand_wave_min(mc, mp);
+            kc[k] = mc;
+            kp[k] = mp;
+            const bool mine = mp != kNone && fp == mp;
+            fc = mine ? 0 : fc;
+            fp = mine ? kNone : fp;
+        }
+        if (cand_less(fc, fp, tc, tp)) { tc = fc; tp = fp; }
+        cand_wave_min(tc, tp);
+        const bool best_only = bounded && hits == 0u;
+        if (best_only && kp[1] != kNone && cand_less(kc[1], kp[1], tc, tp)) { tc = kc[1]; tp = kp[1]; }
+        extras = best_only ? 0u : (uint32_t)(kCandPerGroup - 1);
+        flags = bounded && hits > 0u ? kListOverflow : 0u;
+        oc = kc[0]; op = kp[0];
+#pragma unroll
+        for (int k = 1; k < kCandPerGroup; ++k) { oc = tid == kListHead + k - 1 ? kc[k] : oc; op = tid == kListHead + k - 1 ? kp[k] : op; }
+        if (tid >= kListHead + (int)extras) { oc = 0; op = kNone; }
+    }
+    if (tid == 1) { oc = tc; op = tp; }
+    if (tid == 2) { oc = (int64_t)extras; op = flags; }
+    const int records = (kListHead + (int)extras + 3) & ~3;
+    if (tid < records) store_record_system(slots + (size_t)blockIdx.x * kListRecords + tid, oc, op, tag);
+}
+
 constexpr int kPiRegCompare = 20;
 constexpr int kPiRegBitmapMax = 4096;
 constexpr int kPiRegBitmapWords = 4096;
@@ -804,6 +877,8 @@
     __shared__ uint32_t hkey[kCandHash];
     __shared__ __attribute__((aligned(8))) int64_t hval[kCandHash];
     __shared__ uint32_t s_timeout;
+    __shared__ uint32_t s_hits;
+    __shared__ Cand s_hit[kListHits + 1];
     __shared__ uint32_t sp_mask[TILES * kCandThreads], sp_val[TILES * kCandThreads];
     const int tid = threadIdx.x, nt = (int)blockDim.x;
     int my_i[TILES];
@@ -820,6 +895,7 @@
     for (int i = tid; i < kShiftBits / 32; i += nt) { bitmap[i] = 0u; vmap[i] = 0u; }
     for (int i = tid; i < kCandHash; i += nt) hkey[i] = kHashEmpty;
     for (int i = tid; i < TILES * kCandThreads; i += nt) { sp_mask[i] = 0u; sp_val[i] = 0u; }
+    if (tid == 0) s_hits = 0u;
     __syncthreads();
     auto post_state = [&](int arc, uint32_t val) {
         const int local = arc - p.base;
@@ -845,12 +921,15 @@
         return stage_lines<4>(lm + kStage, p.mb.mailbox, my_unit, shift_base, n_a, first_a, n_v, first_v, seq);
     };
     for (;;) {
-        const bool timed_out = poll_request<kShHdrApplySub>(my_unit, last, last_sub, [](uint32_t c) { return c == kCmdApply || c == kCmdApplyRuns; },
+        const bool timed_out = poll_request<kShHdrApplySub>(my_unit, last, last_sub,
+                                                            [](uint32_t c) { return (c & kShCmdMask) == kCmdApply || (c & kShCmdMask) == kCmdApplyRuns; },
                                                             idle_since, p.mb, lm, s_timeout);
-        const uint32_t seq = lm[kHdrSeq], cmd = lm[kHdrCmd], sub = lm[kShHdrApplySub];
-        const int n_val = clamp_count((int)lm[kShHdrValues], p.mb.max_pi), n_st = clamp_count((int)lm[kHdrStates], p.mb.max_st);
+        const uint32_t seq = lm[kHdrSeq], cmd_word = lm[kHdrCmd], cmd = cmd_word & kShCmdMask, sub = lm[kShHdrApplySub];
+        const int n_val = clamp_count((int)lm[kShHdrValues], p.mb.max_pi), n_st = clamp_count((int)(cmd_word >> kShCmdStatesShift), p.mb.max_st);
         const bool apply_only = cmd == kCmdApply || cmd == kCmdApplyRuns;
-        const bool ranges = apply_only ? cmd == kCmdApplyRuns : lm[kShHdrRuns] == 1u;
+        const bool bounded = !apply_only && (cmd_word & kShCmdBound) != 0u;
+        const int64_t bound = (int64_t)(((uint64_t)lm[kShHdrBound + 1] << 32) | lm[kShHdrBound]);
+        const bool ranges = apply_only ? cmd == kCmdApplyRuns : (cmd_word & kShCmdRuns) != 0u;
         const int per_line = ranges ? kShiftPairsPerLine : kShiftNodesPerLine;
         const int n_shift = apply_only ? 0 : clamp_count((int)lm[kShHdrShift], max_shift_lines * per_line);
         const int shift_lines = clamp_count(apply_only ? (int)lm[kShHdrShift] : (n_shift + per_line - 1) / per_line, max_shift_lines);
@@ -1086,24 +1165,62 @@
             }
         }
         const uint64_t t_patched = blockIdx.x == 0 ? __builtin_amdgcn_s_memrealtime() : 0;
+        auto key_c = [&](int t, int j) -> int64_t {
+            const int st = (int)(int8_t)(mine[t].st4 >> (8 * j));
+            const int64_t dd = (int64_t)mine[t].c.v[j] + (int64_t)ps[t][j] - (int64_t)pt[t][j];
+            return st > 0 ? dd : (st < 0 ? -dd : 0);
+        };
+        uint32_t hit_base = 0;
+        if (bounded) {
+            uint32_t wave_hits = 0;
+#pragma unroll
+            for (int t = 0; t < TILES; ++t)
+#pragma unroll
+                for (int j = 0; j < 4; ++j) {
+                    const int64_t rc = key_c(t, j);
+                    wave_hits += (uint32_t)__popcll(__ballot(rc < 0 && rc < bound));
+                }
+            if ((tid & 63) == 0 && wave_hits > 0) hit_base = atomicAdd(&s_hits, wave_hits);
+            hit_base = (uint32_t)__builtin_amdgcn_readfirstlane((int)hit_base);
+        }
+        __syncthreads();
+        const uint32_t hits = bounded ? s_hits : 0u;
+        const bool listed = hits >= 1u && hits <= (uint32_t)kListHits + 1u;
         int64_t c1 = 0, c2 = 0;
         uint32_t p1 = kNone, p2 = kNone;
-#pragma unroll
-        for (int t = 0; t < TILES; ++t)
-#pragma unroll
-            for (int j = 0; j < 4; ++j) {
-                const int st = (int)(int8_t)(mine[t].st4 >> (8 * j));
-                const int64_t dd = (int64_t)mine[t].c.v[j] + (int64_t)ps[t][j] - (int64_t)pt[t][j];
-                const int64_t rc = st > 0 ? dd : (st < 0 ? -dd : 0);
-                const uint32_t e = (uint32_t)(p.base + my_i[t] + j);
-                const bool b1 = rc < c1;
-                const bool b2 = !b1 && rc < c2;
-                c2 = b1 ? c1 : (b2 ? rc : c2);
-                p2 = b1 ? p1 : (b2 ? e : p2);
-                c1 = b1 ? rc : c1;
-                p1 = b1 ? e : p1;
-            }
-        publish_candidates(c1, p1, c2, p2, p.slots, seq);
+        if (listed) {
+            uint32_t at = hit_base;
+#pragma unroll
+            for (int t = 0; t < TILES; ++t)
+#pragma unroll
+                for (int j = 0; j < 4; ++j) {
+                    const int64_t rc = key_c(t, j);
+                    const uint32_t e = (uint32_t)(p.base + my_i[t] + j);
+                    const bool hit = rc < 0 && rc < bound;
+                    const uint64_t b = __ballot(hit);
+                    const uint32_t before = __builtin_amdgcn_mbcnt_hi((uint32_t)(b >> 32), __builtin_amdgcn_mbcnt_lo((uint32_t)b, 0u));
+                    if (hit && at + before < (uint32_t)kListHits + 1u) s_hit[at + before] = Cand{rc, e};
+                    at += (uint32_t)__popcll(b);
+                    const bool other = !hit && rc < c1;
+                    c1 = other ? rc : c1;
+                    p1 = other ? e : p1;
+                }
+        } else {
+#pragma unroll
+            for (int t = 0; t < TILES; ++t)
+#pragma unroll
+                for (int j = 0; j < 4; ++j) {
+                    const int64_t rc = key_c(t, j);
+                    const uint32_t e = (uint32_t)(p.base + my_i[t] + j);
+                    const bool b1 = rc < c1;
+                    const bool b2 = !b1 && rc < c2;
+                    c2 = b1 ? c1 : (b2 ? rc : c2);
+                    p2 = b1 ? p1 : (b2 ? e : p2);
+                    c1 = b1 ? rc : c1;
+                    p1 = b1 ? e : p1;
+                }
+        }
+        publish_list(listed, bounded, hits, c1, p1, c2, p2, s_hit, s_hits, p.slots, seq);
         if (bits_set) {
             for (int i = tid; i < kShiftBits / 32; i += nt) bitmap[i] = 0u;
             bits_set = false;
diff --git a/mincostflow_amd/csrc/mailbox.hip.h b/mincostflow_amd/csrc/mailbox.hip.h
--- a/mincostflow_amd/csrc/mailbox.hip.h
+++ b/mincostflow_amd/csrc/mailbox.hip.h
@@ -42,9 +42,15 @@
     kHdrApplySub = 14,
     kShHdrValues = 2,
     kShHdrShift = 3,
-    kShHdrRuns = 4,
+    kShHdrBound = 4,
     kShHdrApplySub = 4,
     kShHdrSigma = 13,
+};
+enum : uint32_t {
+    kShCmdMask = 0xFFu,
+    kShCmdRuns = 1u << 8,
+    kShCmdBound = 1u << 9,
+    kShCmdStatesShift = 16,
 };
 
 struct MailboxParams {
diff --git a/mincostflow_amd/network_simplex.py b/mincostflow_amd/network_simplex.py
--- a/mincostflow_amd/network_simplex.py
+++ b/mincostflow_amd/network_simplex.py
@@ -1139,6 +1139,20 @@
     def stats(self) -> dict:
         s = L.EngineStats(); L.check(L.lib().mcf_engine_get_stats(self._h, C.byref(s))); return s.as_dict()
 
+    BOUND_AUTO, BOUND_NONE, BOUND_FIXED = 0, 1, 2
+
+    def candidate_list_control(self, mode: int = 0, bound: int = 0, target: int = 0):
+        L.check(L.lib().mcf_engine_candidate_list_control(self._h, mode, bound, target))
+
+    def candidate_list(self) -> dict:
+        n, tk, ta, ep = C.c_int32(), C.c_int64(), C.c_uint32(), C.c_uint32()
+        arcs, keys = np.zeros(1, np.uint32), np.zeros(1, np.int64)
+        L.check(L.lib().mcf_engine_candidate_list(self._h, 0, arcs, keys, C.byref(n), C.byref(tk), C.byref(ta), C.byref(ep)))
+        arcs, keys = np.zeros(max(1, n.value), np.uint32), np.zeros(max(1, n.value), np.int64)
+        L.check(L.lib().mcf_engine_candidate_list(self._h, n.value, arcs, keys, C.byref(n), C.byref(tk), C.byref(ta), C.byref(ep)))
+        return {"arcs": arcs[:n.value].astype(np.int64), "keys": keys[:n.value], "threshold_key": tk.value,
+                "threshold_arc": None if ta.value == 0xFFFFFFFF else ta.value, "epoch": ep.value}
+
     def park(self):
         L.check(L.lib().mcf_engine_park(self._h))
 
```

Result: no change. 303,700 (-0.2%).
